# radiusxyz/delay-encryption-in-halo2

Measured on AMD Instinct MI355X. Metric: pallas_msm_mpoints_per_s_at_2^20, higher is better.
Workload: dtype u256; 1 GPU; 1 x MSM(2^20, pallas) + 1 x NTT(2^20, pasta_fp) per step per GPU, uniform scalars, SRS tables resident; configs_index=1, steps_in_flight=4, parallelism=single GPU, attempts=1

## Files before the change

### bindings/rust/dehalo-sys/src/lib.rs

```rust
#![allow(non_camel_case_types, non_upper_case_globals, clippy::too_many_arguments)]
#![no_std]

pub use core::ffi::{c_char, c_int, c_void};

pub type dehalo_status = c_int;
pub const DEHALO_OK: dehalo_status = 0;
pub const DEHALO_ERR_INVALID: dehalo_status = -1;
pub const DEHALO_ERR_NO_DEVICE: dehalo_status = -2;
pub const DEHALO_ERR_OOM: dehalo_status = -3;
pub const DEHALO_ERR_HIP: dehalo_status = -4;
pub const DEHALO_ERR_UNSUPPORTED: dehalo_status = -5;
pub const DEHALO_ERR_NOT_IN_TABLE: dehalo_status = -6;
pub const DEHALO_ERR_SHUFFLE: dehalo_status = -7;

pub type dehalo_curve = c_int;
pub const DEHALO_CURVE_BN254_G1: dehalo_curve = 0;
pub const DEHALO_CURVE_PALLAS: dehalo_curve = 1;
pub const DEHALO_CURVE_VESTA: dehalo_curve = 2;

pub type dehalo_field = c_int;
pub const DEHALO_FIELD_BN254_FR: dehalo_field = 0;
pub const DEHALO_FIELD_BN254_FQ: dehalo_field = 1;
pub const DEHALO_FIELD_PASTA_FP: dehalo_field = 2;
pub const DEHALO_FIELD_PASTA_FQ: dehalo_field = 3;
// ... 376 lines not shown
    pub fn dehalo_eval_polynomial_device(ctx: *mut dehalo_ctx, field: c_int, d_coeffs: *const u64, len: usize, stride_elems: usize, batch: usize, point: *const u64, d_out: *mut u64, stream: *mut c_void) -> c_int;
    pub fn dehalo_eval_polynomial_multi_device(ctx: *mut dehalo_ctx, field: c_int, d_polys: *const *const u64, count: usize, len: usize, points: *const u64, num_points: u32, d_out: *mut u64, stream: *mut c_void) -> c_int;
    pub fn dehalo_eval_polynomial_multi_masked_device(ctx: *mut dehalo_ctx, field: c_int, d_polys: *const *const u64, count: usize, len: usize, points: *const u64, num_points: u32, wanted: *const u8, d_out: *mut u64, stream: *mut c_void) -> c_int;
    pub fn dehalo_eval_polynomial_points_device(ctx: *mut dehalo_ctx, field: c_int, d_polys: *const *const u64, count: usize, len: usize, points: *const u64, num_points: u32, wanted: *const u32, d_out: *mut u64, stream: *mut c_void) -> c_int;
    pub fn dehalo_batch_invert(ctx: *mut dehalo_ctx, field: c_int, values: *mut u64, len: usize) -> c_int;
    pub fn dehalo_batch_invert_device(ctx: *mut dehalo_ctx, field: c_int, d_values: *mut u64, len: usize, stream: *mut c_void) -> c_int;
    pub fn dehalo_prefix_product_device(ctx: *mut dehalo_ctx, field: c_int, d_in: *const u64, len: usize, d_out: *mut u64, stream: *mut c_void) -> c_int;
    pub fn dehalo_grand_product(ctx: *mut dehalo_ctx, field: c_int, num: *const u64, den: *const u64, len: usize, z: *mut u64) -> c_int;
    pub fn dehalo_grand_product_device(ctx: *mut dehalo_ctx, field: c_int, d_num: *const u64, d_den: *const u64, len: usize, d_z: *mut u64, stream: *mut c_void) -> c_int;
    pub fn dehalo_grand_product_batch_device(ctx: *mut dehalo_ctx, field: c_int, d_num: *const u64, d_den: *const u64, len: usize, batch: usize, stride_elems: usize, d_z: *mut u64, stream: *mut c_void) -> c_int;
    pub fn dehalo_lincomb_device(ctx: *mut dehalo_ctx, field: c_int, d_cols: *const *const u64, coefs: *const u64, count: usize, len: usize, d_out: *mut u64, sub_const: *const u64, stream: *mut c_void) -> c_int;
    pub fn dehalo_scale_device(ctx: *mut dehalo_ctx, field: c_int, d_a: *mut u64, len: usize, pattern: *const u64, period: u32, d_factor: *const u64, stream: *mut c_void) -> c_int;
    pub fn dehalo_kate_division(ctx: *mut dehalo_ctx, field: c_int, a: *const u64, len: usize, point: *const u64, q: *mut u64) -> c_int;
    pub fn dehalo_kate_division_device(ctx: *mut dehalo_ctx, field: c_int, d_a: *const u64, len: usize, point: *const u64, d_q: *mut u64, stream: *mut c_void) -> c_int;
    pub fn dehalo_kate_division_batch_device(ctx: *mut dehalo_ctx, field: c_int, d_a: *const *const u64, len: usize, points: *const u64, d_q: *const *mut u64, count: usize, stream: *mut c_void) -> c_int;
    pub fn dehalo_vanishing_quotient_batch_device(ctx: *mut dehalo_ctx, field: c_int, d_a: *const *const u64, len: usize, points: *const *const u64, num_points: *const u32, d_q: *const *mut u64, count: usize, stream: *mut c_void) -> c_int;
    pub fn dehalo_convert_form_device(ctx: *mut dehalo_ctx, field: c_int, d_in: *const u64, d_out: *mut u64, n: usize, to_internal: c_int, stream: *mut c_void) -> c_int;
    pub fn dehalo_coset_ntt_form_device(ctx: *mut dehalo_ctx, field: c_int, d_coeffs: *const u64, log_n: u32, d_ext_out: *mut u64, log_ext: u32, omega_ext: *const u64, zeta: *const u64, batch: usize, form_flags: u32, stream: *mut c_void) -> c_int;
    pub fn dehalo_coset_intt_form_device(ctx: *mut dehalo_ctx, field: c_int, d_a: *mut u64, log_ext: u32, omega_ext_inv: *const u64, ext_n_inv: *const u64, zeta: *const u64, batch: usize, form_flags: u32, stream: *mut c_void) -> c_int;
    pub fn dehalo_graph_create(ctx: *mut dehalo_ctx, field: c_int, constants: *const u64, num_constants: u32, rotations: *const i32, num_rotations: u32, calcs: *const dehalo_calculation, num_calcs: u32, horner_parts: *const dehalo_source, num_horner_parts: u32, num_intermediates: u32, out: *mut *mut dehalo_graph) -> c_int;
    pub fn dehalo_graph_release(ctx: *mut dehalo_ctx, graph: *mut dehalo_graph) -> c_int;
    pub fn dehalo_graph_evaluate_device(ctx: *mut dehalo_ctx, graph: *const dehalo_graph, input: *const dehalo_eval_inputs, log_rows: u32, rot_scale: u32, d_previous: *const u64, d_out: *mut u64, stream: *mut c_void) -> c_int;
    pub fn dehalo_graph_evaluate_batch_device(ctx: *mut dehalo_ctx, graphs: *const *const dehalo_graph, count: u32, input: *const dehalo_eval_inputs, log_rows: u32, rot_scale: u32, d_outs: *const *mut u64, stream: *mut c_void) -> c_int;
    pub fn dehalo_permutation_h_device(ctx: *mut dehalo_ctx, field: c_int, input: *const dehalo_perm_inputs, log_rows: u32, rot_scale: u32, d_values: *mut u64, stream: *mut c_void) -> c_int;
    pub fn dehalo_lookup_h_device(ctx: *mut dehalo_ctx, field: c_int, input: *const dehalo_lookup_inputs, log_rows: u32, rot_scale: u32, d_values: *mut u64, stream: *mut c_void) -> c_int;
    pub fn dehalo_lookup_h_batch_device(ctx: *mut dehalo_ctx, field: c_int, input: *const dehalo_lookup_inputs, count: u32, log_rows: u32, rot_scale: u32, d_values: *mut u64, stream: *mut c_void) -> c_int;
    pub fn dehalo_shuffle_h_batch_device(ctx: *mut dehalo_ctx, field: c_int, input: *const dehalo_shuffle_inputs, count: u32, log_rows: u32, rot_scale: u32, d_values: *mut u64, stream: *mut c_void) -> c_int;
    pub fn dehalo_params_create(ctx: *mut dehalo_ctx, curve: c_int, k: u32, g: *const u64, g_lagrange: *const u64, g2: *const u8, s_g2: *const u8, out: *mut *mut dehalo_params) -> c_int;
    pub fn dehalo_params_setup(ctx: *mut dehalo_ctx, curve: c_int, k: u32, s: *const u64, out: *mut *mut dehalo_params) -> c_int;
    pub fn dehalo_params_ipa_create(ctx: *mut dehalo_ctx, curve: c_int, k: u32, g: *const u64, g_lagrange: *const u64, w: *const u64, u: *const u64, out: *mut *mut dehalo_params) -> c_int;
    pub fn dehalo_params_ipa_from_g(ctx: *mut dehalo_ctx, curve: c_int, k: u32, g: *const u64, w: *const u64, u: *const u64, out: *mut *mut dehalo_params) -> c_int;
    pub fn dehalo_params_ipa_size(params: *const dehalo_params) -> usize;
    pub fn dehalo_params_ipa_write(params: *const dehalo_params, out: *mut u8, cap: usize) -> c_int;
    pub fn dehalo_params_ipa_read(ctx: *mut dehalo_ctx, curve: c_int, bytes: *const u8, len: usize, out: *mut *mut dehalo_params) -> c_int;
    pub fn dehalo_params_scheme(params: *const dehalo_params) -> c_int;
    pub fn dehalo_params_fixed_base(params: *const dehalo_params) -> *const dehalo_fixed_base;
    pub fn dehalo_params_read(ctx: *mut dehalo_ctx, curve: c_int, bytes: *const u8, len: usize, out: *mut *mut dehalo_params) -> c_int;
    pub fn dehalo_params_size(params: *const dehalo_params) -> usize;
    pub fn dehalo_params_write(params: *const dehalo_params, out: *mut u8, cap: usize) -> c_int;
    pub fn dehalo_params_release(ctx: *mut dehalo_ctx, params: *mut dehalo_params) -> c_int;
    pub fn dehalo_params_commit_device(ctx: *mut dehalo_ctx, params: *const dehalo_params, d_polys: *const u64, batch: usize, lagrange: c_int, d_out_affine: *mut u64, stream: *mut c_void) -> c_int;
    pub fn dehalo_keygen(ctx: *mut dehalo_ctx, params: *const dehalo_params, cs: *const dehalo_constraint_system, fixed: *const u64, permutation_mapping: *const u64, selectors: *const *const u8, num_selectors: u32, flags: u32, out: *mut *mut dehalo_pk) -> c_int;
    pub fn dehalo_pk_read(ctx: *mut dehalo_ctx, curve: c_int, cs: *const dehalo_constraint_system, bytes: *const u8, len: usize, num_selectors: u32, out: *mut *mut dehalo_pk) -> c_int;
    pub fn dehalo_pk_size(pk: *const dehalo_pk) -> usize;
    pub fn dehalo_pk_write(ctx: *mut dehalo_ctx, pk: *const dehalo_pk, out: *mut u8, cap: usize) -> c_int;
    pub fn dehalo_vk_size(pk: *const dehalo_pk) -> usize;
    pub fn dehalo_vk_write(pk: *const dehalo_pk, out: *mut u8, cap: usize) -> c_int;
    pub fn dehalo_pk_set_transcript_repr(pk: *mut dehalo_pk, repr: *const u64) -> c_int;
    pub fn dehalo_pk_get_transcript_repr(pk: *const dehalo_pk, repr: *mut u64) -> c_int;
    pub fn dehalo_pk_info(pk: *const dehalo_pk, out: *mut u32) -> c_int;
    pub fn dehalo_pk_phases(pk: *const dehalo_pk, out: *mut u32) -> c_int;
    pub fn dehalo_pk_release(ctx: *mut dehalo_ctx, pk: *mut dehalo_pk) -> c_int;
    pub fn dehalo_rng_scalars(rng: *mut dehalo_rng, field: c_int, skip: u64, out: *mut u64, count: usize) -> c_int;
    pub fn dehalo_transcript_create(curve: c_int, out: *mut *mut dehalo_transcript) -> c_int;
    pub fn dehalo_transcript_common_scalar(t: *mut dehalo_transcript, scalar: *const u64) -> c_int;
    pub fn dehalo_transcript_write_scalar(t: *mut dehalo_transcript, scalar: *const u64) -> c_int;
    pub fn dehalo_transcript_write_point(t: *mut dehalo_transcript, affine_xy: *const u64) -> c_int;
    pub fn dehalo_transcript_squeeze_challenge(t: *mut dehalo_transcript, out: *mut u64) -> c_int;
    pub fn dehalo_transcript_len(t: *const dehalo_transcript) -> usize;
    pub fn dehalo_transcript_finalize(t: *const dehalo_transcript, out: *mut u8, cap: usize) -> c_int;
    pub fn dehalo_transcript_release(t: *mut dehalo_transcript);
    pub fn dehalo_ipa_open(ctx: *mut dehalo_ctx, params: *const dehalo_params, d_poly: *const u64, blind: *const u64, x3: *const u64, rng: *mut dehalo_rng, transcript: *mut dehalo_transcript) -> c_int;
    pub fn dehalo_prover_create(ctx: *mut dehalo_ctx, side_ctx: *mut dehalo_ctx, params: *const dehalo_params, pk: *const dehalo_pk, out: *mut *mut dehalo_prover) -> c_int;
    pub fn dehalo_prover_create_multi(ctx: *mut dehalo_ctx, side_ctx: *mut dehalo_ctx, params: *const dehalo_params, pk: *const dehalo_pk, num_circuits: u32, out: *mut *mut dehalo_prover) -> c_int;
    pub fn dehalo_prover_release(prover: *mut dehalo_prover) -> c_int;
    pub fn dehalo_prover_set_multiopen(prover: *mut dehalo_prover, multiopen: c_int) -> c_int;
    pub fn dehalo_prover_proof_size(prover: *const dehalo_prover) -> usize;
    pub fn dehalo_create_proof(prover: *mut dehalo_prover, advice: *const u64, instances: *const *const u64, instance_lens: *const usize, num_instance_columns: u32, rng: *mut dehalo_rng, transcript: *mut dehalo_transcript, flags: u32) -> c_int;
    pub fn dehalo_create_proof_multi(prover: *mut dehalo_prover, advice: *const *const u64, instances: *const *const u64, instance_lens: *const usize, num_instance_columns: u32, num_circuits: u32, rng: *mut dehalo_rng, transcript: *mut dehalo_transcript, flags: u32) -> c_int;
    pub fn dehalo_create_proof_phased(prover: *mut dehalo_prover, func: dehalo_advice_fn, user: *mut c_void, instances: *const *const u64, instance_lens: *const usize, num_instance_columns: u32, rng: *mut dehalo_rng, transcript: *mut dehalo_transcript, flags: u32) -> c_int;
    pub fn dehalo_check_witness(ctx: *mut dehalo_ctx, pk: *const dehalo_pk, advice: *const u64, instances: *const *const u64, instance_lens: *const usize, num_instance_columns: u32, permutation_mapping: *const u64, flags: u32, failures: *mut dehalo_check_failure, cap: usize, report: *mut dehalo_check_report) -> c_int;
    pub fn dehalo_check_witness_challenges(ctx: *mut dehalo_ctx, pk: *const dehalo_pk, advice: *const u64, instances: *const *const u64, instance_lens: *const usize, num_instance_columns: u32, permutation_mapping: *const u64, flags: u32, challenges: *const u64, num_challenges: u32, failures: *mut dehalo_check_failure, cap: usize, report: *mut dehalo_check_report) -> c_int;
    pub fn dehalo_prover_set_shard(prover: *mut dehalo_prover, rank: u32, world: u32, gather: dehalo_gather_fn, user: *mut c_void) -> c_int;
    pub fn dehalo_prover_last_timings(prover: *const dehalo_prover, out: *mut f64) -> c_int;
    pub fn dehalo_create_proofs(provers: *const *mut dehalo_prover, num_provers: u32, advice: *const *const u64, count: u32, rngs: *mut dehalo_rng, flags: u32, proofs_out: *const *mut u8, proof_cap: usize, proof_lens: *mut usize) -> c_int;
    pub fn dehalo_synthesize(input: *const dehalo_circuit_inputs, advice: *mut u64, fixed: *mut u64, mapping: *mut u64, selectors: *const *mut u8, info: *mut dehalo_synthesis_info) -> c_int;
    pub fn dehalo_create_proof_circuit(prover: *mut dehalo_prover, input: *const dehalo_circuit_inputs, info: *mut dehalo_synthesis_info, instances: *const *const u64, instance_lens: *const usize, num_instance_columns: u32, rng: *mut dehalo_rng, transcript: *mut dehalo_transcript) -> c_int;
    pub fn dehalo_create_proofs_circuit(provers: *const *mut dehalo_prover, num_provers: u32, inputs: *const dehalo_circuit_inputs, count: u32, rngs: *mut dehalo_rng, proofs_out: *const *mut u8, proof_cap: usize, proof_lens: *mut usize) -> c_int;
    pub fn dehalo_product_terms_device(ctx: *mut dehalo_ctx, field: c_int, input: *const dehalo_product_inputs, n: usize, d_num: *mut u64, d_den: *mut u64, stride_elems: usize, stream: *mut c_void) -> c_int;
    pub fn dehalo_timing_enable(ctx: *mut dehalo_ctx, on: c_int) -> c_int;
    pub fn dehalo_timing_reset(ctx: *mut dehalo_ctx) -> c_int;
    pub fn dehalo_timing_get(ctx: *mut dehalo_ctx, kernel_id: c_int, total_ms: *mut f64, count: *mut u64) -> c_int;
    pub fn dehalo_msm_last_shape(ctx: *mut dehalo_ctx, out: *mut u32) -> c_int;
    pub fn dehalo_field_info(field: c_int, out: *mut u64) -> c_int;
    pub fn dehalo_version() -> *const c_char;
}

pub const DEHALO_SYS_FUNCTIONS: usize = 132;
```

### delay-encryption-in-halo2_amd/_lib.py

```python
from __future__ import annotations

import ctypes as C
import os
import threading
from typing import Tuple, Optional, Sequence

import numpy as np

_HERE = os.path.dirname(os.path.abspath(__file__))
_LIB = None

SYMBOLS = [
    "dehalo_version", "dehalo_ctx_create", "dehalo_ctx_create_with_priority", "dehalo_ctx_destroy", "dehalo_last_error", "dehalo_ctx_synchronize", "dehalo_download", "dehalo_upload", "dehalo_ctx_stream", "dehalo_ctx_set_tuning",
    "dehalo_bases_register", "dehalo_bases_release", "dehalo_bases_len", "dehalo_bases_info",
    "dehalo_msm", "dehalo_msm_batch", "dehalo_msm_device", "dehalo_msm_device_affine", "dehalo_msm_last_shape", "dehalo_lookup_h_batch_device", "dehalo_product_terms_device", "dehalo_best_multiexp", "dehalo_to_affine", "dehalo_to_affine_device", "dehalo_point_sum_device",
    "dehalo_ntt", "dehalo_ntt_device", "dehalo_intt_scaled", "dehalo_coset_ntt", "dehalo_coset_intt",
    "dehalo_intt_scaled_device", "dehalo_lagrange_to_coeff_device", "dehalo_coset_ntt_device", "dehalo_coset_intt_device",
    "dehalo_field_op", "dehalo_field_op_device", "dehalo_timing_enable", "dehalo_timing_reset", "dehalo_timing_get",
    "dehalo_eval_polynomial", "dehalo_eval_polynomial_device", "dehalo_eval_polynomial_multi_device", "dehalo_eval_polynomial_multi_masked_device", "dehalo_eval_polynomial_points_device", "dehalo_batch_invert", "dehalo_batch_invert_device",
    "dehalo_prefix_product_device", "dehalo_grand_product", "dehalo_grand_product_device", "dehalo_grand_product_batch_device",
    "dehalo_permute_expression_pair", "dehalo_permute_expression_pair_device", "dehalo_permute_expression_pair_batch_device", "dehalo_permute_expression_pair_ptrs_device", "dehalo_permute_expression_pair_distinct_device", "dehalo_permute_expression_pair_ptrs_deferred_device",
    "dehalo_convert_form_device", "dehalo_coset_ntt_form_device", "dehalo_coset_intt_form_device",
    "dehalo_lincomb_device", "dehalo_scale_device", "dehalo_kate_division", "dehalo_kate_division_device", "dehalo_kate_division_batch_device", "dehalo_vanishing_quotient_batch_device",
    "dehalo_params_create", "dehalo_params_setup", "dehalo_bases_register_device", "dehalo_params_read", "dehalo_params_size", "dehalo_params_write", "dehalo_params_release", "dehalo_params_commit_device",
    "dehalo_create_proof_circuit", "dehalo_create_proofs_circuit", "dehalo_keygen", "dehalo_pk_read", "dehalo_pk_size", "dehalo_pk_write", "dehalo_vk_size", "dehalo_vk_write", "dehalo_pk_set_transcript_repr",
    "dehalo_pk_get_transcript_repr", "dehalo_pk_info", "dehalo_pk_release", "dehalo_rng_scalars", "dehalo_field_info", "dehalo_synthesize",
    "dehalo_transcript_create", "dehalo_transcript_common_scalar", "dehalo_transcript_write_scalar", "dehalo_transcript_write_point",
    "dehalo_transcript_squeeze_challenge", "dehalo_transcript_len", "dehalo_transcript_finalize", "dehalo_transcript_release",
    "dehalo_prover_create", "dehalo_prover_release", "dehalo_create_proof", "dehalo_prover_set_shard", "dehalo_prover_last_timings", "dehalo_create_proofs", "dehalo_prover_set_multiopen",
    "dehalo_params_ipa_create", "dehalo_params_scheme", "dehalo_generator_collapse_device", "dehalo_ipa_open", "dehalo_blind_commitments_device", "dehalo_prover_proof_size",
    "dehalo_g_to_lagrange_device", "dehalo_params_ipa_from_g", "dehalo_params_ipa_size", "dehalo_params_ipa_write", "dehalo_params_ipa_read",
    "dehalo_fixed_base_create", "dehalo_fixed_base_release", "dehalo_fixed_base_mul_device", "dehalo_fixed_base_blind_device", "dehalo_params_fixed_base",
    "dehalo_graph_create", "dehalo_graph_release", "dehalo_graph_evaluate_device", "dehalo_graph_evaluate_batch_device", "dehalo_permutation_h_device", "dehalo_lookup_h_device",
    "dehalo_check_witness", "dehalo_check_witness_challenges", "dehalo_create_proof_phased", "dehalo_pk_phases",
    "dehalo_prover_create_multi", "dehalo_create_proof_multi", "dehalo_shuffle_h_batch_device",
]

K_MSM_ACCUMULATE, K_MSM_SORT, K_MSM_REDUCE, K_NTT_PASS, K_POLY, K_EVAL_H = 0, 1, 2, 3, 4, 5


class CSource(C.Structure):
    _fields_ = [("kind", C.c_uint32), ("index", C.c_uint32), ("rotation", C.c_uint32)]


class CCalculation(C.Structure):
    _fields_ = [("op", C.c_uint32), ("a", CSource), ("b", CSource), ("parts_begin", C.c_uint32), ("parts_len", C.c_uint32), ("target", C.c_uint32)]


class CEvalInputs(C.Structure):
    _fields_ = [("fixed", C.POINTER(C.c_void_p)), ("num_fixed", C.c_uint32), ("advice", C.POINTER(C.c_void_p)), ("num_advice", C.c_uint32),
                ("instance", C.POINTER(C.c_void_p)), ("num_instance", C.c_uint32), ("challenges", C.c_void_p), ("num_challenges", C.c_uint32),
                ("beta", C.c_void_p), ("gamma", C.c_void_p), ("theta", C.c_void_p), ("y", C.c_void_p), ("form_flags", C.c_uint32)]


class CPermInputs(C.Structure):
    _fields_ = [("z", C.POINTER(C.c_void_p)), ("num_sets", C.c_uint32), ("columns", C.POINTER(C.c_void_p)), ("sigma", C.POINTER(C.c_void_p)),
                ("num_columns", C.c_uint32), ("chunk_len", C.c_uint32), ("last_rotation", C.c_int32),
                ("l0", C.c_void_p), ("l_last", C.c_void_p), ("l_active_row", C.c_void_p),
                ("beta", C.c_void_p), ("gamma", C.c_void_p), ("y", C.c_void_p), ("delta", C.c_void_p), ("beta_zeta", C.c_void_p), ("extended_omega", C.c_void_p),
                ("form_flags", C.c_uint32)]


class CLookupInputs(C.Structure):
    _fields_ = [("product_coset", C.c_void_p), ("permuted_input_coset", C.c_void_p), ("permuted_table_coset", C.c_void_p), ("table_value", C.c_void_p),
                ("l0", C.c_void_p), ("l_last", C.c_void_p), ("l_active_row", C.c_void_p), ("beta", C.c_void_p), ("gamma", C.c_void_p), ("y", C.c_void_p),
                ("form_flags", C.c_uint32)]


class CShuffleInputs(C.Structure):
    _fields_ = [("product_coset", C.c_void_p), ("input_value", C.c_void_p), ("shuffle_value", C.c_void_p),
                ("l0", C.c_void_p), ("l_last", C.c_void_p), ("l_active_row", C.c_void_p), ("y", C.c_void_p), ("form_flags", C.c_uint32)]


class CExprNode(C.Structure):
    _fields_ = [("kind", C.c_uint32), ("a", C.c_uint32), ("b", C.c_uint32), ("rotation", C.c_int32)]


class CColumnQuery(C.Structure):
    _fields_ = [("kind", C.c_uint32), ("index", C.c_uint32), ("rotation", C.c_int32)]


class CConstraintSystem(C.Structure):
    _fields_ = [("num_advice", C.c_uint32), ("num_fixed", C.c_uint32), ("num_instance", C.c_uint32), ("minimum_degree", C.c_uint32),
                ("nodes", C.POINTER(CExprNode)), ("num_nodes", C.c_uint32), ("constants", C.c_void_p), ("num_constants", C.c_uint32),
                ("gates", C.POINTER(C.c_uint32)), ("num_gates", C.c_uint32), ("lookup_lens", C.POINTER(C.c_uint32)), ("num_lookups", C.c_uint32),
                ("lookup_inputs", C.POINTER(C.c_uint32)), ("lookup_tables", C.POINTER(C.c_uint32)),
                ("permutation_columns", C.POINTER(CColumnQuery)), ("num_permutation_columns", C.c_uint32),
                ("advice_queries", C.POINTER(CColumnQuery)), ("num_advice_queries", C.c_uint32),
                ("fixed_queries", C.POINTER(CColumnQuery)), ("num_fixed_queries", C.c_uint32),
                ("instance_queries", C.POINTER(CColumnQuery)), ("num_instance_queries", C.c_uint32),
                ("advice_phases", C.c_void_p), ("challenge_phases", C.c_void_p), ("num_challenges", C.c_uint32),
                ("shuffle_lens", C.POINTER(C.c_uint32)), ("shuffle_inputs", C.POINTER(C.c_uint32)), ("shuffle_tables", C.POINTER(C.c_uint32)), ("num_shuffles", C.c_uint32)]


class CCircuitInputs(C.Structure):
    _fields_ = [("circuit", C.c_uint32), ("k", C.c_uint32), ("bits_len", C.c_uint32), ("exp_bits", C.c_uint32), ("n", C.c_void_p), ("x", C.c_void_p), ("e", C.c_uint64),
                ("message", C.c_void_p), ("message_len", C.c_uint32), ("key", C.c_void_p), ("t", C.c_uint32), ("rate", C.c_uint32), ("r_f", C.c_uint32), ("r_p", C.c_uint32)]


class CSynthesisInfo(C.Structure):
    _fields_ = [("rsa_rows", C.c_uint64), ("total_rows", C.c_uint64), ("rsa_result", C.c_uint64 * 128), ("cipher", C.c_uint64 * 12), ("cipher_len", C.c_uint32)]


RNG_FILL_FN = C.CFUNCTYPE(C.c_int, C.c_void_p, C.POINTER(C.c_uint64), C.c_size_t, C.c_uint64)
GATHER_FN = C.CFUNCTYPE(C.c_int, C.c_void_p, C.POINTER(C.c_uint64), C.c_uint32, C.POINTER(C.c_uint32), C.POINTER(C.c_uint32), C.c_uint32)
ADVICE_FN = C.CFUNCTYPE(C.c_int, C.c_void_p, C.c_uint32, C.POINTER(C.c_uint64), C.c_uint32, C.POINTER(C.c_void_p))


class CRng(C.Structure):
    _fields_ = [("kind", C.c_int), ("pcg_state", C.c_uint64 * 2), ("pcg_inc", C.c_uint64 * 2), ("fill", RNG_FILL_FN), ("user", C.c_void_p)]


class CProductInputs(C.Structure):
    _fields_ = [("columns", C.POINTER(C.c_void_p)), ("sigma", C.POINTER(C.c_void_p)), ("num_columns", C.c_uint32), ("chunk_len", C.c_uint32), ("omega_powers", C.c_void_p),
                ("beta", C.c_void_p), ("gamma", C.c_void_p), ("delta", C.c_void_p), ("set_factors", C.c_void_p), ("compressed_input", C.POINTER(C.c_void_p)),
                ("compressed_table", C.POINTER(C.c_void_p)), ("permuted_input", C.POINTER(C.c_void_p)), ("permuted_table", C.POINTER(C.c_void_p)), ("num_lookups", C.c_uint32)]


class CCheckFailure(C.Structure):
    _fields_ = [("kind", C.c_uint32), ("index", C.c_uint32), ("row", C.c_uint32), ("reserved", C.c_uint32)]


class CCheckReport(C.Structure):
    _fields_ = [("gate_failures", C.c_uint64), ("lookup_failures", C.c_uint64), ("copy_failures", C.c_uint64), ("rows", C.c_uint64), ("lookup_inputs", C.c_uint64),
                ("cells_in_cycles", C.c_uint64), ("written", C.c_uint64), ("shuffle_failures", C.c_uint64), ("shuffle_inputs", C.c_uint64)]


class DehaloError(RuntimeError):
    def __init__(self, code: int, msg: str):
        super().__init__("dehalo error %d: %s" % (code, msg))
        self.code = code


def library_path() -> str:
    return os.environ.get("DEHALO_LIBRARY") or os.path.join(_HERE, "libdehalo.so")


def load_library():
    global _LIB
    if _LIB is not None:
        return _LIB
    path = library_path()
    if not os.path.exists(path):
        raise DehaloError(-2, "libdehalo.so is not built (run `make` or __graft_entry__.build()); there is no CPU fallback")
    try:
        import torch
    except Exception:
        pass
    lib = C.CDLL(path)
    P, sz, u32, u64p = C.c_void_p, C.c_size_t, C.c_uint32, C.c_void_p
    lib.dehalo_version.restype = C.c_char_p
    lib.dehalo_last_error.restype = C.c_char_p
    lib.dehalo_last_error.argtypes = [P]
    lib.dehalo_ctx_create.argtypes = [C.c_int, C.POINTER(P)]
    lib.dehalo_ctx_create_with_priority.argtypes = [C.c_int, C.c_int, C.POINTER(P)]
    lib.dehalo_ctx_destroy.argtypes = [P]
    lib.dehalo_ctx_destroy.restype = None
    lib.dehalo_ctx_synchronize.argtypes = [P]
    lib.dehalo_download.argtypes = [P, P, C.c_size_t, P]
    lib.dehalo_upload.argtypes = [P, P, C.c_size_t, P]
    lib.dehalo_ctx_set_tuning.argtypes = [P, C.c_char_p, C.c_int]
    lib.dehalo_ctx_stream.argtypes = [P]
    lib.dehalo_ctx_stream.restype = C.c_void_p
    lib.dehalo_bases_register.argtypes = [P, C.c_int, u64p, sz, sz, C.c_int, C.c_int, C.POINTER(P)]
    lib.dehalo_bases_release.argtypes = [P, P]
    lib.dehalo_bases_len.argtypes = [P]
    lib.dehalo_bases_len.restype = sz
    lib.dehalo_bases_info.argtypes = [P, C.POINTER(C.c_uint32), C.POINTER(C.c_uint32), C.POINTER(C.c_int)]
    lib.dehalo_msm.argtypes = [P, P, u64p, sz, u64p]
    lib.dehalo_msm_batch.argtypes = [P, P, C.POINTER(C.c_void_p), sz, sz, u64p]
    lib.dehalo_msm_device.argtypes = [P, P, u64p, sz, sz, u64p, P]
    lib.dehalo_msm_device_affine.argtypes = [P, P, u64p, sz, sz, u64p, u64p, P]
    lib.dehalo_msm_last_shape.argtypes = [P, C.POINTER(C.c_uint32)]
    lib.dehalo_best_multiexp.argtypes = [P, C.c_int, u64p, u64p, sz, u64p]
    lib.dehalo_to_affine.argtypes = [P, C.c_int, u64p, sz, u64p]
    lib.dehalo_to_affine_device.argtypes = [P, C.c_int, u64p, sz, u64p, P]
    lib.dehalo_generator_collapse_device.argtypes = [P, C.c_int, u64p, sz, u64p, u64p, P]
    lib.dehalo_blind_commitments_device.argtypes = [P, C.c_int, u64p, u64p, sz, u64p, P]
    lib.dehalo_point_sum_device.argtypes = [P, C.c_int, u64p, sz, u64p, P]
    lib.dehalo_fixed_base_create.argtypes = [P, C.c_int, u64p, C.POINTER(P)]
    lib.dehalo_fixed_base_release.argtypes = [P, P]
    lib.dehalo_fixed_base_mul_device.argtypes = [P, P, u64p, sz, u64p, P]
    lib.dehalo_fixed_base_blind_device.argtypes = [P, P, u64p, u64p, sz, P]
    lib.dehalo_params_fixed_base.argtypes = [P]
    lib.dehalo_params_fixed_base.restype = C.c_void_p
    lib.dehalo_ntt.argtypes = [P, C.c_int, u64p, u32, u64p]
    lib.dehalo_ntt_device.argtypes = [P, C.c_int, u64p, u32, u64p, sz, P]
    lib.dehalo_intt_scaled.argtypes = [P, C.c_int, u64p, u32, u64p, u64p]
    lib.dehalo_coset_ntt.argtypes = [P, C.c_int, u64p, u32, u64p, u32, u64p, u64p]
    lib.dehalo_coset_intt.argtypes = [P, C.c_int, u64p, u32, u64p, u64p, u64p]
    lib.dehalo_intt_scaled_device.argtypes = [P, C.c_int, u64p, u32, u64p, u64p, sz, P]
    if hasattr(lib, "dehalo_lagrange_to_coeff_device"):
        lib.dehalo_lagrange_to_coeff_device.argtypes = [P, C.c_int, u64p, u64p, u32, u64p, u64p, sz, P]
    lib.dehalo_coset_ntt_device.argtypes = [P, C.c_int, u64p, u32, u64p, u32, u64p, u64p, sz, P]
    lib.dehalo_coset_intt_device.argtypes = [P, C.c_int, u64p, u32, u64p, u64p, u64p, sz, P]
    lib.dehalo_field_op.argtypes = [P, C.c_int, C.c_int, u64p, u64p, u64p, sz]
    lib.dehalo_field_op_device.argtypes = [P, C.c_int, C.c_int, u64p, u64p, u64p, sz, P]
    lib.dehalo_eval_polynomial.argtypes = [P, C.c_int, u64p, sz, u64p, u64p]
    lib.dehalo_eval_polynomial_device.argtypes = [P, C.c_int, u64p, sz, sz, sz, u64p, u64p, P]
    lib.dehalo_eval_polynomial_multi_device.argtypes = [P, C.c_int, C.POINTER(C.c_void_p), sz, sz, u64p, u32, u64p, P]
    lib.dehalo_eval_polynomial_points_device.argtypes = [P, C.c_int, C.POINTER(C.c_void_p), sz, sz, u64p, u32, C.POINTER(C.c_uint32), u64p, P]
    if hasattr(lib, "dehalo_eval_polynomial_multi_masked_device"):
        lib.dehalo_eval_polynomial_multi_masked_device.argtypes = [P, C.c_int, C.POINTER(C.c_void_p), sz, sz, u64p, u32, C.c_char_p, u64p, P]
    lib.dehalo_batch_invert.argtypes = [P, C.c_int, u64p, sz]
    lib.dehalo_batch_invert_device.argtypes = [P, C.c_int, u64p, sz, P]
    lib.dehalo_prefix_product_device.argtypes = [P, C.c_int, u64p, sz, u64p, P]
    lib.dehalo_grand_product.argtypes = [P, C.c_int, u64p, u64p, sz, u64p]
    lib.dehalo_grand_product_device.argtypes = [P, C.c_int, u64p, u64p, sz, u64p, P]
    lib.dehalo_grand_product_batch_device.argtypes = [P, C.c_int, u64p, u64p, sz, sz, sz, u64p, P]
    lib.dehalo_permute_expression_pair.argtypes = [P, C.c_int, u64p, u64p, sz, u64p, u64p]
    lib.dehalo_permute_expression_pair_device.argtypes = [P, C.c_int, u64p, u64p, sz, u64p, u64p, P]
    lib.dehalo_permute_expression_pair_batch_device.argtypes = [P, C.c_int, u64p, u64p, sz, sz, sz, u64p, u64p, P]
    if hasattr(lib, "dehalo_permute_expression_pair_ptrs_deferred_device"):
        lib.dehalo_permute_expression_pair_ptrs_deferred_device.argtypes = [P, C.c_int, C.POINTER(C.c_void_p), C.POINTER(C.c_void_p), sz, sz, C.POINTER(C.c_void_p), C.POINTER(C.c_void_p), P, P]
    if hasattr(lib, "dehalo_permute_expression_pair_distinct_device"):
        lib.dehalo_permute_expression_pair_distinct_device.argtypes = [P, C.c_int, C.POINTER(C.c_void_p), C.POINTER(C.c_void_p), sz, sz, C.POINTER(C.c_void_p), C.POINTER(C.c_void_p),
                                                                       C.POINTER(C.c_void_p), C.POINTER(C.c_void_p), C.POINTER(C.c_uint32), P, P]
    if hasattr(lib, "dehalo_permute_expression_pair_ptrs_device"):
        lib.dehalo_permute_expression_pair_ptrs_device.argtypes = [P, C.c_int, C.POINTER(C.c_void_p), C.POINTER(C.c_void_p), sz, sz, C.POINTER(C.c_void_p), C.POINTER(C.c_void_p), P]
    lib.dehalo_lincomb_device.argtypes = [P, C.c_int, C.POINTER(C.c_void_p), u64p, sz, sz, u64p, u64p, P]
    lib.dehalo_scale_device.argtypes = [P, C.c_int, u64p, sz, u64p, u32, u64p, P]
    lib.dehalo_kate_division.argtypes = [P, C.c_int, u64p, sz, u64p, u64p]
    lib.dehalo_kate_division_device.argtypes = [P, C.c_int, u64p, sz, u64p, u64p, P]
    lib.dehalo_kate_division_batch_device.argtypes = [P, C.c_int, C.POINTER(C.c_void_p), sz, u64p, C.POINTER(C.c_void_p), sz, P]
    lib.dehalo_vanishing_quotient_batch_device.argtypes = [P, C.c_int, C.POINTER(C.c_void_p), sz, C.POINTER(C.c_void_p), C.POINTER(C.c_uint32), C.POINTER(C.c_void_p), sz, P]
    lib.dehalo_convert_form_device.argtypes = [P, C.c_int, u64p, u64p, sz, C.c_int, P]
    lib.dehalo_coset_ntt_form_device.argtypes = [P, C.c_int, u64p, u32, u64p, u32, u64p, u64p, sz, u32, P]
    lib.dehalo_coset_intt_form_device.argtypes = [P, C.c_int, u64p, u32, u64p, u64p, u64p, sz, u32, P]
    lib.dehalo_graph_create.argtypes = [P, C.c_int, u64p, u32, C.POINTER(C.c_int32), u32, C.POINTER(CCalculation), u32, C.POINTER(CSource), u32, u32, C.POINTER(P)]
    lib.dehalo_graph_release.argtypes = [P, P]
    lib.dehalo_graph_evaluate_device.argtypes = [P, P, C.POINTER(CEvalInputs), u32, u32, u64p, u64p, P]
    lib.dehalo_graph_evaluate_batch_device.argtypes = [P, C.POINTER(C.c_void_p), u32, C.POINTER(CEvalInputs), u32, u32, C.POINTER(C.c_void_p), P]
    lib.dehalo_permutation_h_device.argtypes = [P, C.c_int, C.POINTER(CPermInputs), u32, u32, u64p, P]
    lib.dehalo_lookup_h_device.argtypes = [P, C.c_int, C.POINTER(CLookupInputs), u32, u32, u64p, P]
    if hasattr(lib, "dehalo_product_terms_device"):
        lib.dehalo_product_terms_device.argtypes = [P, C.c_int, C.POINTER(CProductInputs), sz, u64p, u64p, sz, P]
    lib.dehalo_lookup_h_batch_device.argtypes = [P, C.c_int, C.POINTER(CLookupInputs), u32, u32, u32, u64p, P]
    lib.dehalo_shuffle_h_batch_device.argtypes = [P, C.c_int, C.POINTER(CShuffleInputs), u32, u32, u32, u64p, P]
    PP = C.POINTER(P)
    lib.dehalo_params_create.argtypes = [P, C.c_int, u32, u64p, u64p, P, P, PP]
    lib.dehalo_params_setup.argtypes = [P, C.c_int, u32, u64p, PP]
    lib.dehalo_bases_register_device.argtypes = [P, C.c_int, u64p, C.c_size_t, C.c_int, C.c_int, PP]
    lib.dehalo_params_read.argtypes = [P, C.c_int, P, sz, PP]
    lib.dehalo_params_size.argtypes = [P]
    lib.dehalo_params_size.restype = sz
    lib.dehalo_params_write.argtypes = [P, P, sz]
    lib.dehalo_params_release.argtypes = [P, P]
    lib.dehalo_params_commit_device.argtypes = [P, P, u64p, sz, C.c_int, u64p, P]
    lib.dehalo_params_ipa_create.argtypes = [P, C.c_int, u32, u64p, u64p, u64p, u64p, PP]
    lib.dehalo_params_scheme.argtypes = [P]
    lib.dehalo_g_to_lagrange_device.argtypes = [P, C.c_int, u64p, u32, u64p, P]
    lib.dehalo_params_ipa_from_g.argtypes = [P, C.c_int, u32, u64p, u64p, u64p, PP]
    lib.dehalo_params_ipa_size.argtypes = [P]
    lib.dehalo_params_ipa_size.restype = sz
    lib.dehalo_params_ipa_write.argtypes = [P, P, sz]
    lib.dehalo_params_ipa_read.argtypes = [P, C.c_int, P, sz, PP]
# ... 112 lines not shown
            self.handle = None

    def __enter__(self):
        return self

    def __exit__(self, *exc):
        self.close()

    def _check(self, rc: int):
        if rc != 0:
            raise DehaloError(rc, self.lib.dehalo_last_error(self.handle).decode())

    def synchronize(self):
        self._check(self.lib.dehalo_ctx_synchronize(self.handle))

    def download(self, d_src: int, count: int, width: int = 4) -> np.ndarray:
        out = np.empty((count, width), dtype=np.uint64)
        self._check(self.lib.dehalo_download(self.handle, d_src, out.nbytes, out.ctypes.data))
        return out

    def upload(self, host, dtype=None):
        import torch

        a = np.ascontiguousarray(host)
        assert a.dtype.itemsize in (8, 4, 1), "upload: 64-bit words (field elements, indices), 32-bit words or bytes"
        if dtype is None:
            dtype = {8: torch.int64, 4: torch.int32, 1: torch.uint8}[a.dtype.itemsize]
        out = torch.empty(a.shape, dtype=dtype, device=torch.device("cuda", self.device))
        self._check(self.lib.dehalo_upload(self.handle, a.ctypes.data, a.nbytes, out.data_ptr()))
        return out

    def download_tensor(self, t) -> np.ndarray:
        assert t.is_contiguous() and t.element_size() == 8
        out = np.empty(tuple(t.shape), dtype=np.uint64)
        self._check(self.lib.dehalo_download(self.handle, t.data_ptr(), out.nbytes, out.ctypes.data))
        return out

    def set_tuning(self, key: str, value: int):
        self._check(self.lib.dehalo_ctx_set_tuning(self.handle, key.encode(), value))

    def torch_stream_obj(self):
        self.torch_stream()
        return self._tstream

    def torch_stream(self):
        import torch

        if getattr(self, "_tstream", None) is None:
            self._tstream = torch.cuda.ExternalStream(self.lib.dehalo_ctx_stream(self.handle))
        return torch.cuda.stream(self._tstream)

    def register_bases(self, curve: int, affine_xy, window_bits: int = 0, precompute: bool = True) -> Bases:
        a = _u64(affine_xy, 8)
        h = C.c_void_p()
        self._check(self.lib.dehalo_bases_register(self.handle, curve, _ptr(a), a.shape[0], 64, window_bits, int(precompute), C.byref(h)))
        return Bases(self, h, curve, a.shape[0])

    def msm(self, bases: Bases, scalars) -> np.ndarray:
        s = _u64(scalars, 4)
        out = np.zeros(12, dtype=np.uint64)
        self._check(self.lib.dehalo_msm(self.handle, bases.handle, _ptr(s), s.shape[0], _ptr(out)))
        return out

    def msm_batch(self, bases: Bases, columns: Sequence) -> np.ndarray:
        cols = [_u64(c, 4) for c in columns]
        n = cols[0].shape[0] if cols else 0
        assert all(c.shape[0] == n for c in cols)
        ptrs = (C.c_void_p * len(cols))(*[c.ctypes.data for c in cols])
        out = np.zeros((len(cols), 12), dtype=np.uint64)
        self._check(self.lib.dehalo_msm_batch(self.handle, bases.handle, ptrs, n, len(cols), _ptr(out)))
        return out

    def msm_device(self, bases: Bases, d_scalars: int, length: int, batch: int, d_out: int, stream: int = 0):
        self._check(self.lib.dehalo_msm_device(self.handle, bases.handle, d_scalars, length, batch, d_out, stream or None))

    def msm_device_affine(self, bases: Bases, d_scalars: int, length: int, batch: int, d_out_jacobian: int, d_out_affine: int, stream: int = 0):
        self._check(self.lib.dehalo_msm_device_affine(self.handle, bases.handle, d_scalars, length, batch, d_out_jacobian or None, d_out_affine, stream or None))

    def msm_last_shape(self) -> dict:
        out = (C.c_uint32 * 6)()
        self._check(self.lib.dehalo_msm_last_shape(self.handle, out))
        return {"merge_light": out[0], "merge_32": out[1], "merge_wave": out[2], "merge_block": out[3], "points_per_lane": out[4], "pairs": out[5]}

    def best_multiexp(self, curve: int, scalars, affine_xy) -> np.ndarray:
        s, a = _u64(scalars, 4), _u64(affine_xy, 8)
        if s.shape[0] != a.shape[0]:
            raise ValueError("best_multiexp: coeffs.len() != bases.len()")
        out = np.zeros(12, dtype=np.uint64)
        self._check(self.lib.dehalo_best_multiexp(self.handle, curve, _ptr(s), _ptr(a), s.shape[0], _ptr(out)))
        return out

    def to_affine(self, curve: int, jacobian) -> np.ndarray:
        j = _u64(jacobian, 12)
        out = np.zeros((j.shape[0], 8), dtype=np.uint64)
        self._check(self.lib.dehalo_to_affine(self.handle, curve, _ptr(j), j.shape[0], _ptr(out)))
        return out

    def point_sum_device(self, curve: int, d_jacobian: int, count: int, d_out: int, stream: int = 0):
        self._check(self.lib.dehalo_point_sum_device(self.handle, curve, d_jacobian, count, d_out, stream or None))

    def generator_collapse_device(self, curve: int, d_affine: int, length: int, challenge, d_out: int, stream: int = 0):
        ch = np.ascontiguousarray(challenge, dtype=np.uint64).reshape(4)
        self._check(self.lib.dehalo_generator_collapse_device(self.handle, curve, d_affine, length, ch.ctypes.data, d_out, stream or None))

    def g_to_lagrange(self, curve: int, d_g: int, k: int, d_out: Optional[int] = None, stream: int = 0):
        self._check(self.lib.dehalo_g_to_lagrange_device(self.handle, curve, d_g, k, d_g if d_out is None else d_out, stream or None))

    def blind_commitments_device(self, curve: int, d_jacobian: int, d_blinds: int, count: int, d_w_affine: int, stream: int = 0):
        self._check(self.lib.dehalo_blind_commitments_device(self.handle, curve, d_jacobian or None, d_blinds or None, count, d_w_affine or None, stream or None))

    def fixed_base(self, curve: int, affine_xy) -> FixedBase:
        a = np.ascontiguousarray(affine_xy, dtype=np.uint64).reshape(8)
        h = C.c_void_p()
        self._check(self.lib.dehalo_fixed_base_create(self.handle, curve, _ptr(a), C.byref(h)))
        return FixedBase(self, h, curve)

    def to_affine_device(self, curve: int, d_jacobian: int, count: int, d_affine: int, stream: int = 0):
        self._check(self.lib.dehalo_to_affine_device(self.handle, curve, d_jacobian, count, d_affine, stream or None))

    def ntt(self, field: int, a, log_n: int, omega) -> np.ndarray:
        a = np.array(a, dtype=np.uint64).reshape(-1, 4)
        if a.shape[0] != 1 << log_n:
            raise ValueError("best_fft: a.len() != 1 << log_n")
        self._check(self.lib.dehalo_ntt(self.handle, field, _ptr(a), log_n, _ptr(_u64(omega, 4))))
        return a

    def intt_scaled(self, field: int, a, log_n: int, omega_inv, n_inv) -> np.ndarray:
        a = np.array(a, dtype=np.uint64).reshape(-1, 4)
        if a.shape[0] != 1 << log_n:
            raise ValueError("a.len() != 1 << log_n")
        self._check(self.lib.dehalo_intt_scaled(self.handle, field, _ptr(a), log_n, _ptr(_u64(omega_inv, 4)), _ptr(_u64(n_inv, 4))))
        return a

    def coset_ntt(self, field: int, coeffs, log_n: int, log_ext: int, omega_ext, zeta) -> np.ndarray:
        c = _u64(coeffs, 4)
        if c.shape[0] != 1 << log_n:
            raise ValueError("coeffs.len() != 1 << log_n")
        out = np.zeros((1 << log_ext, 4), dtype=np.uint64)
        self._check(self.lib.dehalo_coset_ntt(self.handle, field, _ptr(c), log_n, _ptr(out), log_ext, _ptr(_u64(omega_ext, 4)), _ptr(_u64(zeta, 4))))
        return out

    def coset_intt(self, field: int, a, log_ext: int, omega_ext_inv, ext_n_inv, zeta) -> np.ndarray:
        a = np.array(a, dtype=np.uint64).reshape(-1, 4)
        if a.shape[0] != 1 << log_ext:
            raise ValueError("a.len() != 1 << log_ext")
        self._check(self.lib.dehalo_coset_intt(self.handle, field, _ptr(a), log_ext, _ptr(_u64(omega_ext_inv, 4)), _ptr(_u64(ext_n_inv, 4)),
                                               _ptr(_u64(zeta, 4))))
        return a

    def ntt_device(self, field: int, d_a: int, log_n: int, omega, batch: int = 1, stream: int = 0):
        self._check(self.lib.dehalo_ntt_device(self.handle, field, d_a, log_n, _ptr(_u64(omega, 4)), batch, stream or None))

    def intt_scaled_device(self, field: int, d_a: int, log_n: int, omega_inv, n_inv, batch: int = 1, stream: int = 0):
        self._check(self.lib.dehalo_intt_scaled_device(self.handle, field, d_a, log_n, _ptr(_u64(omega_inv, 4)), _ptr(_u64(n_inv, 4)), batch, stream or None))

    def lagrange_to_coeff_device(self, field: int, d_values: int, d_coeffs: int, log_n: int, omega_inv, n_inv, batch: int = 1, stream: int = 0):
        self._check(self.lib.dehalo_lagrange_to_coeff_device(self.handle, field, d_values, d_coeffs, log_n, _ptr(_u64(omega_inv, 4)), _ptr(_u64(n_inv, 4)), batch, stream or None))

    def coset_ntt_device(self, field: int, d_coeffs: int, log_n: int, d_ext: int, log_ext: int, omega_ext, zeta, batch: int = 1, stream: int = 0):
        self._check(self.lib.dehalo_coset_ntt_device(self.handle, field, d_coeffs, log_n, d_ext, log_ext, _ptr(_u64(omega_ext, 4)), _ptr(_u64(zeta, 4)), batch,
                                                     stream or None))

    def convert_form_device(self, field: int, d_in: int, d_out: int, n: int, to_internal: bool, stream: int = 0):
        self._check(self.lib.dehalo_convert_form_device(self.handle, field, d_in, d_out, n, int(to_internal), stream or None))

    def coset_ntt_form_device(self, field: int, d_coeffs: int, log_n: int, d_ext: int, log_ext: int, omega_ext, zeta, batch: int, form_flags: int, stream: int = 0):
# ... 282 lines not shown
```

### delay-encryption-in-halo2_amd/csrc/capi.hip

```cpp
#include <algorithm>
#include <atomic>
#include <initializer_list>

#include <map>
#include <memory>

#include "evalh_types.hpp"
#include "hostfield.hpp"
#include "internal.hpp"
#include "msm_plan.hpp"

namespace {

const FieldOps* field_ops(int field) {
    static const FieldOps* const ops[] = {&bn254_fr_field_ops(), &bn254_fq_field_ops(), &pasta_fp_field_ops(), &pasta_fq_field_ops()};
    static_assert(DEHALO_FIELD_BN254_FR == 0 && DEHALO_FIELD_BN254_FQ == 1 && DEHALO_FIELD_PASTA_FP == 2 && DEHALO_FIELD_PASTA_FQ == 3, "field ids");
    return field >= 0 && field < 4 ? ops[field] : nullptr;
}
const CurveOps* curve_ops(int curve) {
    static const CurveOps* const ops[] = {&bn254_curve_ops(), &pallas_curve_ops(), &vesta_curve_ops()};
    static_assert(DEHALO_CURVE_BN254_G1 == 0 && DEHALO_CURVE_PALLAS == 1 && DEHALO_CURVE_VESTA == 2, "curve ids");
    return curve >= 0 && curve < 3 ? ops[curve] : nullptr;
}
int unknown_field(dehalo_ctx* ctx) { return dh_fail(ctx, DEHALO_ERR_INVALID, "unknown field id"); }
// ... 273 lines not shown
        hipDeviceProp_t prop;
        if (hipGetDeviceProperties(&prop, device) != hipSuccess) return DEHALO_ERR_NO_DEVICE;
        if (strncmp(prop.gcnArchName, "gfx950", 6) != 0) return DEHALO_ERR_NO_DEVICE;
        if (hipSetDevice(device) != hipSuccess) return DEHALO_ERR_NO_DEVICE;
        std::unique_ptr<dehalo_ctx> ctx(new dehalo_ctx());
        ctx->device = device;
        ctx->num_cus = prop.multiProcessorCount > 0 ? prop.multiProcessorCount : 256;
        {
            int least = 0, greatest = 0;
            (void)hipDeviceGetStreamPriorityRange(&least, &greatest);
            const int prio = priority > 0 ? greatest : (priority < 0 ? least : 0);
            static const int cu_parts = [] { const char* e = DH_EXPERIMENT_ENV("DEHALO_CU_PARTITION"); return e ? atoi(e) : 0; }();
            static std::atomic<int> cu_next{0};
            hipError_t e;
            hipStream_t st = nullptr;
            if (cu_parts > 1 && cu_parts <= 16) {
                const int part = cu_next.fetch_add(1) % cu_parts, ncu = ctx->num_cus, per = ncu / cu_parts;
                std::vector<uint32_t> mask((ncu + 31) / 32, 0u);
                static const bool interleave = DH_EXPERIMENT_ENV("DEHALO_CU_PARTITION_INTERLEAVE") != nullptr;
                for (int cu = 0; cu < ncu; cu++) {
                    const bool mine = interleave ? (cu % cu_parts) == part : (cu / per) == part;
                    if (mine) mask[cu / 32] |= 1u << (cu % 32);
                }
                e = hipExtStreamCreateWithCUMask(&st, (uint32_t)mask.size(), mask.data());
                if (e == hipSuccess) ctx->num_cus = per;
            } else
            e = priority == 0 ? hipStreamCreateWithFlags(&st, hipStreamNonBlocking)
                              : hipStreamCreateWithPriority(&st, hipStreamNonBlocking, prio);
            if (e != hipSuccess) return DEHALO_ERR_HIP;
            ctx->stream.reset(st);
        }
        if (const char* e = DH_EXPERIMENT_ENV("DEHALO_MSM_ACC_MIN_LAYERS")) ctx->msm_acc_min_layers = std::max(1, std::min(4, atoi(e)));
        if (const char* e = DH_EXPERIMENT_ENV("DEHALO_HOST_SPIN_US")) ctx->host_wait_spin_us = std::max(0, std::min(1000000, atoi(e)));
        if (const char* e = DH_EXPERIMENT_ENV("DEHALO_MSM_ACC_BLOCK")) ctx->msm_acc_block = atoi(e) == 768 ? 768 : 128;
        if (const char* e = DH_EXPERIMENT_ENV("DEHALO_MSM_ACC_POINTS")) ctx->msm_acc_points = std::max(0, std::min(4096, atoi(e)));
        *out = ctx.release();
        return 0;
    });
}

void dehalo_ctx_destroy(dehalo_ctx* ctx) {
    if (!ctx) return;
    (void)hipSetDevice(ctx->device);
    (void)hipDeviceSynchronize();
    delete ctx;
}

const char* dehalo_last_error(const dehalo_ctx* ctx) {
    if (!ctx) return "null context";
    static thread_local std::string copy;
    try {
        std::lock_guard<std::mutex> lk(const_cast<dehalo_ctx*>(ctx)->err_mu);
        copy = ctx->err;
    } catch (...) {
        return "out of host memory copying the last error";
    }
    return copy.c_str();
}

int dehalo_ctx_set_tuning(dehalo_ctx* ctx, const char* key, int value) {
    if (!ctx || !key) return DEHALO_ERR_INVALID;
    return dh_guard(ctx, [&]() -> int {
        std::lock_guard<std::recursive_mutex> lk(ctx->mu);
        if (!strcmp(key, "msm_acc_points")) {
            if (value < 0 || value > 4096) return dh_fail(ctx, DEHALO_ERR_INVALID, "msm_acc_points must be in [0, 4096]");
            ctx->msm_acc_points = value;
            return 0;
        }
        if (!strcmp(key, "msm_acc_waves")) {
            if (value < 1 || value > 4) return dh_fail(ctx, DEHALO_ERR_INVALID, "msm_acc_waves must be in [1, 4]");
            ctx->msm_acc_waves = value;
            return 0;
        }
        if (!strcmp(key, "host_wait_spin_us")) {
            if (value < 0 || value > 1000000) return dh_fail(ctx, DEHALO_ERR_INVALID, "host_wait_spin_us must be in [0, 1000000]");
            ctx->host_wait_spin_us = value;
            return 0;
        }
        if (!strcmp(key, "msm_sort_block")) {
            if (value != 512 && value != 1024) return dh_fail(ctx, DEHALO_ERR_INVALID, "msm_sort_block must be 512 or 1024");
            ctx->msm_sort_block = value;
            return 0;
        }
        if (!strcmp(key, "msm_acc_block")) {
            if (value != 128 && value != 768) return dh_fail(ctx, DEHALO_ERR_INVALID, "msm_acc_block must be 128 or 768");
            ctx->msm_acc_block = value;
            return 0;
        }
        if (!strcmp(key, "ntt_full_table_log")) {
            if (value < 0 || value > 30) return dh_fail(ctx, DEHALO_ERR_INVALID, "ntt_full_table_log must be in [0, 30]");
            ctx->ntt_full_table_log = value;
            return 0;
        }
        return dh_fail(ctx, DEHALO_ERR_INVALID, std::string("unknown tuning key: ") + key);
    });
}

void* dehalo_ctx_stream(dehalo_ctx* ctx) { return ctx ? (void*)ctx->stream.get() : nullptr; }

int dehalo_ctx_synchronize(dehalo_ctx* ctx) {
    if (!ctx) return DEHALO_ERR_INVALID;
    return dh_guard(ctx, [&]() -> int {
        HIP_TRY(ctx, hipStreamSynchronize(ctx->stream.get()));
        return 0;
    });
}

int dehalo_download(dehalo_ctx* ctx, const void* d_src, size_t bytes, void* host_dst) {
    if (!ctx) return DEHALO_ERR_INVALID;
    return dh_guard(ctx, [&]() -> int {
        if ((!d_src || !host_dst) && bytes) return dh_fail(ctx, DEHALO_ERR_INVALID, "download: null argument");
        (void)hipSetDevice(ctx->device);
        if (bytes) TRY(dh_d2h(ctx, host_dst, d_src, bytes, ctx->stream.get()));
        HIP_TRY(ctx, dh_stream_wait(ctx, ctx->stream.get()));
        return 0;
    });
}

int dehalo_upload(dehalo_ctx* ctx, const void* host_src, size_t bytes, void* d_dst) {
    if (!ctx) return DEHALO_ERR_INVALID;
    return dh_guard(ctx, [&]() -> int {
        if ((!host_src || !d_dst) && bytes) return dh_fail(ctx, DEHALO_ERR_INVALID, "upload: null argument");
        (void)hipSetDevice(ctx->device);
        {
            HostPin pin(host_src, bytes);
            TRY(dh_h2d(ctx, d_dst, host_src, bytes, ctx->stream.get()));
            HIP_TRY(ctx, hipStreamSynchronize(ctx->stream.get()));
        }
        return 0;
    });
}

int dehalo_bases_register(dehalo_ctx* ctx, int curve, const uint64_t* affine_xy, size_t n, size_t stride_bytes, int window_bits, int precompute,
                          dehalo_bases** out) {
    return register_entry(ctx, curve, affine_xy, n, stride_bytes, window_bits, precompute, out, false);
}

int dehalo_bases_register_device(dehalo_ctx* ctx, int curve, const uint64_t* d_affine_xy, size_t n, int window_bits, int precompute, dehalo_bases** out) {
    return register_entry(ctx, curve, d_affine_xy, n, 64, window_bits, precompute, out, true);
}

int dehalo_bases_release(dehalo_ctx* ctx, dehalo_bases* bases) {
    if (!ctx || !bases) return DEHALO_ERR_INVALID;
    return dh_guard(ctx, [&] {
        std::lock_guard<std::recursive_mutex> lk(ctx->mu);
        (void)hipSetDevice(ctx->device);
        (void)hipDeviceSynchronize();
        delete bases;
        return 0;
    });
}

size_t dehalo_bases_len(const dehalo_bases* bases) { return bases ? bases->n : 0; }

int dehalo_bases_info(const dehalo_bases* bases, uint32_t* window_bits, uint32_t* windows, int* precomputed) {
    if (!bases) return DEHALO_ERR_INVALID;
    if (window_bits) *window_bits = bases->c;
    if (windows) *windows = bases->W;
    if (precomputed) *precomputed = bases->precomp;
    return 0;
}

int dehalo_msm_device(dehalo_ctx* ctx, const dehalo_bases* bases, const uint64_t* d_scalars, size_t len, size_t batch, uint64_t* d_out_jacobian,
                      void* stream) {
    if (!bases || (!d_scalars && len) || !d_out_jacobian) return dh_fail(ctx, DEHALO_ERR_INVALID, "msm: null argument");
    if (len > bases->n) return dh_fail(ctx, DEHALO_ERR_INVALID, "msm: more scalars than registered bases");
// ... 724 lines not shown
        return dh_fail(ctx, DEHALO_ERR_INVALID, "product_terms: incomplete permutation inputs");
    if (in->num_lookups && (!in->compressed_input || !in->compressed_table || !in->permuted_input || !in->permuted_table))
        return dh_fail(ctx, DEHALO_ERR_INVALID, "product_terms: incomplete lookup inputs");
    if (in->num_columns > 256 || in->num_lookups > 256) return dh_fail(ctx, DEHALO_ERR_INVALID, "product_terms: too many columns");
    if (stride_elems < n) return dh_fail(ctx, DEHALO_ERR_INVALID, "product_terms: stride shorter than the columns");
    return field_device(ctx, field, stream, [&](const FieldOps& f, hipStream_t s) { return f.product_terms(ctx, in, n, (fe*)d_num, (fe*)d_den, stride_elems, s); });
}

int dehalo_lookup_h_batch_device(dehalo_ctx* ctx, int field, const dehalo_lookup_inputs* in, uint32_t count, uint32_t log_rows, uint32_t rot_scale,
                                 uint64_t* d_values, void* stream) {
    if (!in || !d_values || count == 0) return dh_fail(ctx, DEHALO_ERR_INVALID, "lookup_h_batch: null argument");
    if (count > 8) return dh_fail(ctx, DEHALO_ERR_INVALID, "lookup_h_batch: more than 8 lookups in one call");
    for (uint32_t l = 0; l < count; l++) {
        const dehalo_lookup_inputs& q = in[l];
        if (!q.product_coset || !q.permuted_input_coset || !q.permuted_table_coset || !q.table_value || !q.l0 || !q.l_last || !q.l_active_row || !q.beta ||
            !q.gamma || !q.y)
            return dh_fail(ctx, DEHALO_ERR_INVALID, "lookup_h_batch: null argument");
        if (q.l0 != in[0].l0 || q.l_last != in[0].l_last || q.l_active_row != in[0].l_active_row || q.form_flags != in[0].form_flags ||
            memcmp(q.beta, in[0].beta, 32) || memcmp(q.gamma, in[0].gamma, 32) || memcmp(q.y, in[0].y, 32))
            return dh_fail(ctx, DEHALO_ERR_INVALID, "lookup_h_batch: the lookups of one call share l0 / l_last / l_active_row, the challenges and the form flags");
    }
    if (log_rows > 30) return dh_fail(ctx, DEHALO_ERR_INVALID, "lookup_h: log_rows > 30");
    return field_device(ctx, field, stream, [&](const FieldOps& f, hipStream_t s) { return f.lookup_h_batch(ctx, in, count, log_rows, rot_scale, (fe*)d_values, s); });
}

int dehalo_shuffle_h_batch_device(dehalo_ctx* ctx, int field, const dehalo_shuffle_inputs* in, uint32_t count, uint32_t log_rows, uint32_t rot_scale,
                                  uint64_t* d_values, void* stream) {
    if (!in || !d_values || count == 0) return dh_fail(ctx, DEHALO_ERR_INVALID, "shuffle_h_batch: null argument");
    if (count > 8) return dh_fail(ctx, DEHALO_ERR_INVALID, "shuffle_h_batch: more than 8 shuffles in one call");
    for (uint32_t j = 0; j < count; j++) {
        const dehalo_shuffle_inputs& q = in[j];
        if (!q.product_coset || !q.input_value || !q.shuffle_value || !q.l0 || !q.l_last || !q.l_active_row || !q.y)
            return dh_fail(ctx, DEHALO_ERR_INVALID, "shuffle_h_batch: null argument");
        if (q.l0 != in[0].l0 || q.l_last != in[0].l_last || q.l_active_row != in[0].l_active_row || q.form_flags != in[0].form_flags || memcmp(q.y, in[0].y, 32))
            return dh_fail(ctx, DEHALO_ERR_INVALID, "shuffle_h_batch: the shuffles of one call share l0 / l_last / l_active_row, y and the form flags");
    }
    if (log_rows > 30) return dh_fail(ctx, DEHALO_ERR_INVALID, "shuffle_h_batch: log_rows > 30");
    return field_device(ctx, field, stream, [&](const FieldOps& f, hipStream_t s) { return f.shuffle_h_batch(ctx, in, count, log_rows, rot_scale, (fe*)d_values, s); });
}

int dehalo_timing_enable(dehalo_ctx* ctx, int on) {
    if (!ctx) return DEHALO_ERR_INVALID;
    return dh_guard(ctx, [&]() -> int {
        std::lock_guard<std::recursive_mutex> lk(ctx->mu);
        ctx->timing = on != 0;
        return 0;
    });
}

static int timing_collect(dehalo_ctx* ctx) {
    (void)hipSetDevice(ctx->device);
    for (auto& r : ctx->regions) {
        HIP_TRY(ctx, hipEventSynchronize(r.b.get()));
        float ms = 0;
        HIP_TRY(ctx, hipEventElapsedTime(&ms, r.a.get(), r.b.get()));
        ctx->timing_ms[r.kernel_id] += ms;
        ctx->timing_cnt[r.kernel_id] += 1;
    }
    ctx->regions.clear();
    return 0;
}

int dehalo_timing_reset(dehalo_ctx* ctx) {
    if (!ctx) return DEHALO_ERR_INVALID;
    return dh_guard(ctx, [&]() -> int {
        std::lock_guard<std::recursive_mutex> lk(ctx->mu);
        TRY(timing_collect(ctx));
        for (int i = 0; i < DEHALO_K_COUNT; i++) { ctx->timing_ms[i] = 0; ctx->timing_cnt[i] = 0; }
        return 0;
    });
}

int dehalo_timing_get(dehalo_ctx* ctx, int kernel_id, double* total_ms, uint64_t* count) {
    if (!ctx || kernel_id < 0 || kernel_id >= DEHALO_K_COUNT || !total_ms || !count) return DEHALO_ERR_INVALID;
    return dh_guard(ctx, [&]() -> int {
        std::lock_guard<std::recursive_mutex> lk(ctx->mu);
        TRY(timing_collect(ctx));
        *total_ms = ctx->timing_ms[kernel_id];
        *count = ctx->timing_cnt[kernel_id];
        return 0;
    });
}

int dehalo_msm_last_shape(dehalo_ctx* ctx, uint32_t out[6]) {
    if (!ctx || !out) return DEHALO_ERR_INVALID;
    return dh_guard(ctx, [&]() -> int {
        std::lock_guard<std::recursive_mutex> lk(ctx->mu);
        (void)hipSetDevice(ctx->device);
        memset(out, 0, 6 * sizeof(uint32_t));
        if (!ctx->ws_counters.p) return 0;
        HIP_TRY(ctx, hipStreamSynchronize(ctx->stream.get()));
        uint32_t raw[10];
        HIP_TRY(ctx, hipMemcpy(raw, ctx->ws_counters.p, sizeof(raw), hipMemcpyDeviceToHost));
        out[0] = raw[0] + raw[1] + raw[2]; out[1] = raw[3]; out[2] = raw[4]; out[3] = raw[6]; out[4] = raw[8]; out[5] = raw[9];
        return 0;
    });
}

}

int dh_graph_create_roots(dehalo_ctx* ctx, int field, const uint64_t* constants, uint32_t num_constants, const int32_t* rotations, uint32_t num_rotations,
                          const dehalo_calculation* calcs, uint32_t num_calcs, const dehalo_source* horner_parts, uint32_t num_horner_parts, uint32_t num_intermediates,
                          const uint32_t* root_of, uint32_t num_roots, dehalo_graph** out) {
    if (ctx && num_calcs && !root_of) return dh_fail(ctx, DEHALO_ERR_INVALID, "graph_create: null root table");
    return graph_create_impl(ctx, field, constants, num_constants, rotations, num_rotations, calcs, num_calcs, horner_parts, num_horner_parts, num_intermediates, root_of,
                             num_roots, out);
}
```

### delay-encryption-in-halo2_amd/csrc/internal.hpp

```cpp
#pragma once
#include <hip/hip_runtime.h>

#include <algorithm>
#include <cstdint>
#include <cstdlib>
#include <cstring>
#include <map>
#include <chrono>
#include <mutex>
#include <string>
#include <thread>
#include <vector>

#include "../../include/dehalo.h"
#include "ec.cuh"
#include "experiment_env.hpp"
#include "guard.hpp"
#include "owners.hpp"

using DevMem = DevArray<fe>;

struct HostStage {
    static constexpr size_t CHUNK = 4u << 20;
    static constexpr size_t DIRECT_MAX = 64u << 10;
    std::mutex mu;
    Pinned<void> buf[2];
    Event ev[2];
    bool busy[2] = {false, false};
};

struct TwiddleEntry {
    int field;
    uint32_t log_n;
    int form;
    uint64_t omega[4];
    uint64_t len;
    DevMem tw;
};

struct TimedRegion {
    int kernel_id;
    Event a, b;
};

struct dehalo_ctx {
    int device = 0;
    int num_cus = 256;
    Stream stream;
    std::string err;
    std::mutex err_mu;
    std::recursive_mutex mu;
    DevBuf ws_scalars, ws_out, ws_count, ws_counters, ws_off, ws_records, ws_merge_lists, ws_merge_parts, ws_bhist, ws_pcount, ws_pairs, ws_bsum, ws_idx, ws_partial0, ws_buckets,
        ws_contrib, ws_tree, ws_bred_cnt, ws_gsums, ws_ntt_scratch, ws_ntt_io, ws_ntt_io2, ws_fop[3], ws_tmp_bases, ws_poly[5], ws_poly_io[3], ws_evh[4], ws_lookup, ws_gfft, ws_check[3];
    std::vector<TwiddleEntry> twiddles;
    affine_t* msm_affine_out = nullptr;
    int msm_acc_points = 48;
    int msm_acc_waves = 3;
    int host_wait_spin_us = 400;
    int msm_acc_min_layers = 4;
    int msm_sort_block = 1024;
    int msm_acc_block = 128;
    int ntt_full_table_log = 0;
    HostStage stage;
    bool timing = false;
    std::vector<TimedRegion> regions;
    double timing_ms[DEHALO_K_COUNT] = {};
    uint64_t timing_cnt[DEHALO_K_COUNT] = {};
};

struct dehalo_bases {
    int curve;
    size_t n;
    uint32_t c, W;
    int precomp;
    DevArray<affine_t> table;
};

struct dehalo_fixed_base {
    int curve;
    DevArray<affine_t> table;
};

inline int dh_fail(dehalo_ctx* ctx, int code, const char* msg) noexcept {
    if (ctx) try {
        std::lock_guard<std::mutex> lk(ctx->err_mu);
        ctx->err = msg;
    } catch (...) {}
    return code;
}
inline int dh_fail(dehalo_ctx* ctx, int code, const std::string& msg) noexcept { return dh_fail(ctx, code, msg.c_str()); }

template <class Body>
int dh_guard(dehalo_ctx* ctx, Body&& body) noexcept {
    return dh_guard_noting([ctx](const char* msg) { dh_fail(ctx, DEHALO_ERR_INVALID, msg); }, body);
}

inline hipStream_t pick_stream(dehalo_ctx* ctx, void* stream) { return stream ? (hipStream_t)stream : ctx->stream.get(); }
inline hipStream_t dh_ctx_stream(dehalo_ctx* ctx) { return ctx->stream.get(); }

template <class Body>
int dh_device(dehalo_ctx* ctx, void* stream, Body&& body) noexcept {
    if (!ctx) return DEHALO_ERR_INVALID;
    return dh_guard(ctx, [&]() -> int {
        std::lock_guard<std::recursive_mutex> lk(ctx->mu);
        (void)hipSetDevice(ctx->device);
        return body(pick_stream(ctx, stream));
    });
}

inline hipError_t dh_func_lds(dehalo_ctx* ctx, const void* fn, int bytes) {
    static std::mutex mu;
    static std::map<std::pair<int, const void*>, int> have;
    std::lock_guard<std::mutex> lk(mu);
    int& cur = have[std::make_pair(ctx->device, fn)];
    if (cur >= bytes) return hipSuccess;
    const hipError_t e = hipFuncSetAttribute(fn, hipFuncAttributeMaxDynamicSharedMemorySize, bytes);
    if (e == hipSuccess) cur = bytes;
    return e;
}

inline int dh_ensure(dehalo_ctx* ctx, DevBuf& b, size_t bytes) { return b.ensure(ctx, bytes); }

inline bool dh_host_locked(const void* ptr, size_t bytes) {
    {
        HostPinRegistry& reg = host_pin_registry();
        std::lock_guard<std::mutex> lk(reg.mu);
        const uintptr_t a = (uintptr_t)ptr, b = a + bytes;
        for (auto& e : reg.entries)
            if (e.a <= a && b <= e.b) return true;
    }
    hipPointerAttribute_t at;
    if (hipPointerGetAttributes(&at, ptr) == hipSuccess) return at.type == hipMemoryTypeHost;
    (void)hipGetLastError();
    return false;
}

inline int dh_stage_init(dehalo_ctx* ctx) {
    HostStage& st = ctx->stage;
    for (int i = 0; i < 2; i++) {
        if (!st.buf[i]) HIP_TRY(ctx, make_pinned(st.buf[i], HostStage::CHUNK));
        if (!st.ev[i]) HIP_TRY(ctx, make_event(st.ev[i], hipEventDisableTiming));
    }
// ... 203 lines not shown
```

### delay-encryption-in-halo2_amd/csrc/msm.cuh

```cuda
#pragma once
#include <algorithm>
#include <cstdlib>
#include <cstdio>
#include <vector>

#include "ec29.cuh"
#include "internal.hpp"
#include "msm_plan.hpp"

#ifndef MSM_ACC_WAVES_ATTR
#ifdef MSM_ACC_CAP
#define MSM_ACC_WAVES_ATTR __attribute__((amdgpu_waves_per_eu(MSM_ACC_CAP, MSM_ACC_CAP)))
#else
#define MSM_ACC_WAVES_ATTR __attribute__((amdgpu_waves_per_eu(4, 4)))
#endif
#endif
#ifdef MSM_HIST_VGPR64
#define MSM_HIST_ATTR __attribute__((amdgpu_num_vgpr(64)))
#else
#define MSM_HIST_ATTR
#endif

#ifndef MSM_TAIL_PRIO
#define MSM_TAIL_PRIO 0
#endif
FP_DEV void msm_tail_prio() {
#if MSM_TAIL_PRIO > 0
    __builtin_amdgcn_s_setprio(MSM_TAIL_PRIO);
#endif
}

FP_DEV u32 merge2_class(u32 S) { return S <= 2 ? 0u : S <= 4 ? 1u : S <= 8 ? 2u : S <= 64 ? 3u : S <= MERGE2_CHUNK ? 4u : 5u; }

FP_DEV bool fe_is_zero_words(const fe& a) { return (a.v[0] | a.v[1] | a.v[2] | a.v[3] | a.v[4] | a.v[5] | a.v[6] | a.v[7]) == 0; }

template <class FS, class Fn>
FP_DEV void for_each_digit(const fe& mont_scalar, u32 c, u32 w_lo, u32 w_hi, Fn f) {
    if (fe_is_zero_words(mont_scalar)) return;
    fe s = f_from_mont<FS>(mont_scalar);
    u32 bits = 0;
#pragma unroll
    for (int i = 0; i < 8; i++) if (s.v[i]) bits = 32u * i + (32u - (u32)__clz((int)s.v[i]));
    const u32 w_end = min(w_hi, (bits + c - 1) / c + 1);
    const u32 mask = (1u << c) - 1, halfv = 1u << (c - 1);
    u32 carry = 0;
    for (u32 w = 0; w < w_end; w++) {
        u32 raw = (s.v[0] & mask) + carry;
#pragma unroll
        for (int i = 0; i < 7; i++) s.v[i] = (s.v[i] >> c) | (s.v[i + 1] << (32 - c));
        s.v[7] >>= c;
        bool neg = raw > halfv;
        carry = neg ? 1u : 0u;
        u32 mag = neg ? (1u << c) - raw : raw;
        if (mag != 0 && w >= w_lo) f(w, mag - 1, neg);
    }
}

struct DigitStream {
    fe s;
    u32 carry, c, mask, halfv;
    template <class FS>
    FP_DEV void init(const fe& mont_scalar, u32 c_) {
        s = f_from_mont<FS>(mont_scalar);
        c = c_; mask = (1u << c) - 1; halfv = 1u << (c - 1); carry = 0;
    }
    FP_DEV bool exhausted() const { return carry == 0 && fe_is_zero_words(s); }
    FP_DEV void next(u32& bucket, bool& neg) {
        u32 raw = (s.v[0] & mask) + carry;
#pragma unroll
        for (int i = 0; i < 7; i++) s.v[i] = (s.v[i] >> c) | (s.v[i + 1] << (32 - c));
        s.v[7] >>= c;
        neg = raw > halfv;
        carry = neg ? 1u : 0u;
        u32 mag = neg ? (1u << c) - raw : raw;
        bucket = mag - 1;
    }
};

FP_DEV bool wave_value_groups(const fe& s, bool active, u32 lane, u32 max_groups, u32& leader, u32& cnt, u32& rank) {
    unsigned long long rem = __ballot(active);
    leader = lane; cnt = 1; rank = 0;
    for (u32 n = 0; rem; n++) {
        if (n == max_groups) return false;
        const int ld = __ffsll((long long)rem) - 1;
        bool eq = active;
#pragma unroll
        for (int w = 0; w < 8; w++) eq &= s.v[w] == (u32)__shfl((int)s.v[w], ld);
        const unsigned long long m = __ballot(eq);
        if (eq) { leader = (u32)ld; cnt = (u32)__popcll(m); rank = (u32)__popcll(m & ((1ull << lane) - 1)); }
        rem &= ~m;
    }
    return true;
}

template <class FS, bool PACK16>
__global__ __launch_bounds__(MSM_SORT_THREADS) MSM_HIST_ATTR void k_msm_hist(MsmGeom g, const fe* scalars, u32* bh, u32* pc) {
    msm_tail_prio();
    extern __shared__ u32 lhist[];
    const u32 bat = blockIdx.z;
    const u32 w_lo = g.G == 1 ? 0 : blockIdx.y * g.wb, w_hi = g.G == 1 ? g.W : min(g.W, w_lo + g.wb);
    const u32 ng = g.G == 1 ? 1 : w_hi - w_lo, grp0 = g.G == 1 ? 0 : w_lo;
    for (u32 b = threadIdx.x; b < (PACK16 ? ng * g.nb / 2 : ng * g.nb); b += blockDim.x) lhist[b] = 0;
    __syncthreads();
    const fe* sc = scalars + (u64)bat * g.n;
    const u32 per = (g.n + g.slices - 1) / g.slices;
    const u32 beg = blockIdx.x * per, end = min(beg + per, g.n);
    const bool one = g.G == 1;
    for (u32 i0 = beg + threadIdx.x; i0 < end; i0 += 4 * blockDim.x) {
        fe s4[4];
#pragma unroll
        for (int j = 0; j < 4; j++)
            if (i0 + j * blockDim.x < end) s4[j] = f_load(&sc[i0 + j * blockDim.x]);
#pragma unroll
        for (int j = 0; j < 4; j++) {
            const bool valid = i0 + j * blockDim.x < end;
            u32 gl, weight, grank;
            const bool grouped = wave_value_groups(s4[j], valid, threadIdx.x & 63, 4, gl, weight, grank);
            if (!grouped) weight = 1;
            const bool counts = grouped ? valid && (threadIdx.x & 63) == gl : valid;
            if (counts)
                for_each_digit<FS>(s4[j], g.c, w_lo, w_hi, [&](u32 w, u32 bucket, bool) {
                    const u32 slot = (one ? 0u : (w - w_lo) * g.nb) + bucket;
                    if (PACK16) atomicAdd(&lhist[slot >> 1], weight << ((slot & 1u) << 4));
                    else atomicAdd(&lhist[slot], weight);
                });
        }
    }
    __syncthreads();
    const u32 sub = msm_sub_bits(g.c), P = g.nb >> sub;
    for (u32 gi = 0; gi < ng; gi++) {
        const u64 gidx = (u64)bat * g.G + grp0 + gi;
        const u32* lh = lhist + (PACK16 ? gi * g.nb / 2 : gi * g.nb);
        if (PACK16) {
            u32* out = bh + ((gidx * g.slices + blockIdx.x) * g.nb) / 2;
            for (u32 w = threadIdx.x; w < g.nb / 2; w += blockDim.x) out[w] = lh[w];
        } else {
            u32* out = bh + (gidx * g.slices + blockIdx.x) * g.nb;
            for (u32 b = threadIdx.x; b < g.nb; b += blockDim.x) out[b] = lh[b];
        }
        u32* pout = pc + (gidx * g.slices + blockIdx.x) * P;
        const u32 nsub = 1u << sub, lane = threadIdx.x & 63;
        for (u32 q = threadIdx.x >> 6; q < P; q += blockDim.x >> 6) {
            u32 sum = 0;
            if (PACK16) {
                for (u32 w = lane; w < nsub / 2; w += 64) { const u32 x = lh[(q << sub) / 2 + w]; sum += (x & 0xffffu) + (x >> 16); }
            } else {
                for (u32 b = lane; b < nsub; b += 64) sum += lh[(q << sub) + b];
            }
#pragma unroll
            for (int d = 32; d > 0; d >>= 1) sum += __shfl_down(sum, d);
            if (lane == 0) pout[q] = sum;
        }
    }
}

template <bool SRC16>
FP_DEV u32 colscan_one(u32 nb, u32 slices, u32 total_buckets, u32* bh, const unsigned short* src16, u32* count, u32 gb) {
    if (gb >= total_buckets) return 0;
    u32 grp = gb / nb, b = gb - grp * nb;
    u32* col = bh + (u64)grp * slices * nb + b;
    const unsigned short* col16 = SRC16 ? src16 + (u64)grp * slices * nb + b : nullptr;
    u32 run = 0;
    u32 k = 0;
    for (; k + 16 <= slices; k += 16) {
        u32 v[16];
#pragma unroll
        for (int j = 0; j < 16; j++) v[j] = SRC16 ? (u32)col16[(u64)(k + j) * nb] : col[(u64)(k + j) * nb];
#pragma unroll
        for (int j = 0; j < 16; j++) {
            col[(u64)(k + j) * nb] = run;
            run += v[j];
        }
    }
    for (; k < slices; k++) {
        u32 v = SRC16 ? (u32)col16[(u64)k * nb] : col[(u64)k * nb];
        col[(u64)k * nb] = run;
        run += v;
    }
    if (count) count[gb] = run;
    return run;
}
static __global__ __launch_bounds__(SCAN_THREADS) void k_msm_colscan(u32 nb, u32 slices, u32 total_buckets, u32* bh, const unsigned short* bh16, u32* count, u32 blocks_a, u32 P,
                                                                     u32 total_parts, u32* pc, u32* bsum_items, u32* bsum_tasks, u32* merge_counters) {
    msm_tail_prio();
    if (blockIdx.x == 0 && threadIdx.x < MSM_MERGE_COUNTERS) merge_counters[threadIdx.x] = 0;
    if (blockIdx.x >= blocks_a) {
        colscan_one<false>(P, slices, total_parts, pc, nullptr, nullptr, (blockIdx.x - blocks_a) * blockDim.x + threadIdx.x);
        return;
    }
    const u32 gb0 = blockIdx.x * blockDim.x + threadIdx.x;
    const u32 v = bh16 ? colscan_one<true>(nb, slices, total_buckets, bh, bh16, count, gb0) : colscan_one<false>(nb, slices, total_buckets, bh, nullptr, count, gb0);
    u32 si = v, st = v ? 1u : 0u;
#pragma unroll
    for (int d = 32; d > 0; d >>= 1) { si += __shfl_down(si, d); st += __shfl_down(st, d); }
    __shared__ u32 w_i[SCAN_THREADS / 64], w_t[SCAN_THREADS / 64];
    if ((threadIdx.x & 63) == 0) { w_i[threadIdx.x >> 6] = si; w_t[threadIdx.x >> 6] = st; }
    __syncthreads();
    if (threadIdx.x == 0) {
        u32 a = 0, b = 0;
        for (u32 w = 0; w < SCAN_THREADS / 64; w++) { a += w_i[w]; b += w_t[w]; }
        bsum_items[blockIdx.x] = a; bsum_tasks[blockIdx.x] = b;
    }
}

static __global__ __launch_bounds__(SCAN_THREADS) void k_scan_offsets(const u32* cnt, u32 total, const u32* bsum_items, const u32* bsum_tasks, u32 nblocks, u32* geo, u32 resident,
                                                                      u32 lmax, u32 lcap, u32 kmin, u32* off, u32* nrank, u32* rbeg, u32* rend, u32* lists, u32 cap) {
    msm_tail_prio();
    __shared__ u32 s_i[SCAN_THREADS], s_t[SCAN_THREADS];
    __shared__ u32 w4[4][SCAN_THREADS / 64];
    const u32 tid = threadIdx.x, lane = tid & 63, wave = tid >> 6;
    u32 bi = 0, bt = 0, ti = 0;
    for (u32 j = tid; j < nblocks; j += SCAN_THREADS) {
        const u32 a = bsum_items[j];
        ti += a;
        if (j < blockIdx.x) { bi += a; bt += bsum_tasks[j]; }
    }
#pragma unroll
    for (int d = 32; d > 0; d >>= 1) { bi += __shfl_down(bi, d); bt += __shfl_down(bt, d); ti += __shfl_down(ti, d); }
    if (lane == 0) { w4[0][wave] = bi; w4[1][wave] = bt; w4[2][wave] = ti; }
    const u32 idx = blockIdx.x * SCAN_THREADS + tid;
    const u32 vi = idx < total ? cnt[idx] : 0, vt = vi ? 1u : 0u;
    s_i[tid] = vi; s_t[tid] = vt;
    __syncthreads();
    bi = 0; bt = 0; ti = 0;
    for (u32 w = 0; w < SCAN_THREADS / 64; w++) { bi += w4[0][w]; bt += w4[1][w]; ti += w4[2][w]; }
    const u64 M = ti;
    u64 L;
    if (lcap) {
        u64 k = kmin;
        while (M > k * resident * lcap) k += k < 4 ? 1 : 2;
        L = max((u64)4, (M + k * resident - 1) / (k * resident));
    } else {
        const u64 rounds = max((u64)1, (M + (u64)resident * lmax - 1) / ((u64)resident * lmax));
        L = (M + rounds * resident - 1) / (rounds * resident);
        L = min((u64)lmax, max((u64)4, L));
    }
    if (blockIdx.x == 0 && tid == 0) { geo[0] = (u32)L; geo[1] = (u32)M; }
    for (u32 d = 1; d < SCAN_THREADS; d <<= 1) {
        const u32 ai = tid >= d ? s_i[tid - d] : 0, at = tid >= d ? s_t[tid - d] : 0;
        __syncthreads();
        s_i[tid] += ai; s_t[tid] += at;
        __syncthreads();
    }
    const u32 ri = bi + s_i[tid] - vi, rt = bt + s_t[tid] - vt;
    u32 S = 0;
    if (idx < total) {
        off[idx] = ri; nrank[idx] = rt;
        const u32 b0 = (u32)(ri / L) + rt;
        const u32 b1 = vi ? (u32)((ri + vi - 1) / L) + rt + 1 : b0;
        rbeg[idx] = b0;
        rend[idx] = b1;
        S = b1 - b0;
        if (idx + 1 == total) { off[total] = ri + vi; nrank[total] = rt + vt; }
    }
    if (!lists) return;
    u32* counters = geo - MSM_MERGE_COUNTERS;
    const u32 cls = S <= 1 ? 8u : merge2_class(S);
    __shared__ u32 wcnt[5][SCAN_THREADS / 64], cbase[5];
    unsigned long long mine = 0;
    for (u32 c = 0; c < 5; c++) {
        const unsigned long long mask = __ballot(cls == c);
        if (cls == c) mine = mask;
        if (lane == 0) wcnt[c][wave] = (u32)__popcll(mask);
    }
    __syncthreads();
    if (tid < 5) {
        u32 tot = 0;
        for (u32 w = 0; w < SCAN_THREADS / 64; w++) tot += wcnt[tid][w];
        cbase[tid] = tot ? atomicAdd(&counters[tid], tot) : 0u;
    }
    __syncthreads();
    if (cls < 5) {
        u32 pos = cbase[cls] + (u32)__popcll(mine & ((1ull << lane) - 1));
        for (u32 w = 0; w < wave; w++) pos += wcnt[cls][w];
        lists[(size_t)cls * cap + pos] = idx;
    }
    if (cls == 5u) {
        const u32 parts = (S + MERGE2_CHUNK - 1) / MERGE2_CHUNK;
        const u32 slot = atomicAdd(&counters[6], 1u), first = atomicAdd(&counters[5], parts);
        u32* hb = lists + (size_t)6 * cap + 4 * (size_t)slot;
        hb[0] = idx; hb[1] = first; hb[2] = parts; hb[3] = 0;
        for (u32 p = 0; p < parts; p++) {
            lists[(size_t)5 * cap + 2 * (size_t)(first + p)] = slot;
            lists[(size_t)5 * cap + 2 * (size_t)(first + p) + 1] = p;
        }
    }
}

template <class FS>
__global__ __launch_bounds__(MSM_SORT_THREADS) void k_msm_part(MsmGeom g, const fe* scalars, const u32* off, const u32* pc, unsigned long long* pairs, u32 lists) {
    msm_tail_prio();
    extern __shared__ __align__(8) unsigned char part_smem[];
    const u32 bat = blockIdx.z;
    const u32 sub = msm_sub_bits(g.c), P = g.nb >> sub, submask = (1u << sub) - 1;
    const u32 w_lo = g.G == 1 ? 0 : blockIdx.y * g.wb, w_hi = g.G == 1 ? g.W : min(g.W, w_lo + g.wb);
    const u32 ng = g.G == 1 ? 1 : w_hi - w_lo, grp0 = g.G == 1 ? 0 : w_lo;
    const u32 PT = ng * P;
    const bool one = g.G == 1;
    const u32 wave = threadIdx.x >> 6, lane = threadIdx.x & 63, nwaves = blockDim.x >> 6;
    u32* pcur = reinterpret_cast<u32*>(part_smem);
    unsigned char* wbase = part_smem + 4 * lists + (size_t)wave * MSM_PART_WAVE_LDS(lists);
    unsigned long long* stage = reinterpret_cast<unsigned long long*>(wbase);
    u32* lcnt = reinterpret_cast<u32*>(wbase + 512 * 8);
    u32* lbase = lcnt + lists;
    u32* lcur = lbase + lists;
    u32* gbase = lcur + lists;
    unsigned short* stageq = reinterpret_cast<unsigned short*>(gbase + lists);
    for (u32 qq = threadIdx.x; qq < PT; qq += blockDim.x) {
        const u32 gi = qq / P, q = qq - gi * P;
        const u64 gidx = (u64)bat * g.G + grp0 + gi;
        pcur[qq] = off[gidx * g.nb + (q << sub)] + pc[(gidx * g.slices + blockIdx.x) * P + q];
    }
    __syncthreads();
    const fe* sc = scalars + (u64)bat * g.n;
    const u32 per = (g.n + g.slices - 1) / g.slices;
    const u32 beg = blockIdx.x * per, end = min(beg + per, g.n);
    (void)nwaves;
    fe s_next;
    if (beg + wave * 64 + lane < end) s_next = f_load(&sc[beg + wave * 64 + lane]);
    for (u32 i0 = beg + wave * 64; i0 < end; i0 += blockDim.x) {
        const u32 i = i0 + lane;
        const bool have = i < end;
        const fe s_cur = s_next;
        if (i + blockDim.x < end) s_next = f_load(&sc[i + blockDim.x]);
        const bool nonzero = have && !fe_is_zero_words(s_cur);
        const unsigned long long actm = __ballot(nonzero);
        if (actm == 0) continue;
        DigitStream ds;
        if (nonzero) ds.template init<FS>(s_cur, g.c);
        {
            u32 gl, gcnt, grank;
            if (__popcll(actm) > 1 && wave_value_groups(s_cur, nonzero, lane, 4, gl, gcnt, grank)) {
                for (u32 w = 0; w < w_hi; w++) {
                    if (__ballot(nonzero && !ds.exhausted()) == 0) break;
                    u32 bk = 0xffffffffu; bool ng1 = false;
                    if (nonzero) ds.next(bk, ng1);
                    const bool put = nonzero && w >= w_lo && bk != 0xffffffffu;
                    const u32 q = put ? (one ? 0u : (w - w_lo) * P) + (bk >> sub) : 0u;
                    u32 g0 = 0;
                    if (put && lane == gl) g0 = atomicAdd(&pcur[q], gcnt);
                    g0 = (u32)__shfl((int)g0, (int)gl);
                    const u32 tidx = one ? w * g.table_n + i : i;
                    if (put) pairs[g0 + grank] = ((unsigned long long)(bk & submask) << 32) | (tidx | (ng1 ? 0x80000000u : 0u));
                }
                continue;
            }
        }
        for (u32 w0 = 0; w0 < w_hi; w0 += 8) {
            if (__ballot(nonzero && !ds.exhausted()) == 0) break;
            u32 bk[8];
            bool ng8[8];
#pragma unroll
            for (int j = 0; j < 8; j++) {
                bk[j] = 0xffffffffu; ng8[j] = false;
                if (nonzero && w0 + j < w_hi) {
                    ds.next(bk[j], ng8[j]);
                    if (w0 + j < w_lo) bk[j] = 0xffffffffu;
                }
            }
            if (w0 + 8 <= w_lo) continue;
            for (u32 q = lane; q < PT; q += 64) lcnt[q] = 0;
            __builtin_amdgcn_wave_barrier();
#pragma unroll
            for (int j = 0; j < 8; j++)
                if (bk[j] != 0xffffffffu) atomicAdd(&lcnt[(one ? 0u : (w0 + j - w_lo) * P) + (bk[j] >> sub)], 1u);
            __builtin_amdgcn_wave_barrier();
            u32 run = 0;
            for (u32 q0 = 0; q0 < PT; q0 += 64) {
                const u32 q = q0 + lane;
                const u32 v = q < PT ? lcnt[q] : 0;
                u32 x = v;
#pragma unroll
                for (int d = 1; d < 64; d <<= 1) { u32 y = __shfl_up(x, d); if ((int)lane >= d) x += y; }
                if (q < PT) {
                    lbase[q] = run + x - v; lcur[q] = run + x - v;
                    gbase[q] = v ? atomicAdd(&pcur[q], v) : 0u;
                }
                run += __shfl(x, 63);
            }
            __builtin_amdgcn_wave_barrier();
#pragma unroll
            for (int j = 0; j < 8; j++)
                if (bk[j] != 0xffffffffu) {
                    const u32 q = (one ? 0u : (w0 + j - w_lo) * P) + (bk[j] >> sub);
                    const u32 pos = atomicAdd(&lcur[q], 1u);
                    const u32 tidx = one ? (w0 + j) * g.table_n + i : i;
                    stage[pos] = ((unsigned long long)(bk[j] & submask) << 32) | (tidx | (ng8[j] ? 0x80000000u : 0u));
                    stageq[pos] = (unsigned short)q;
                }
            __builtin_amdgcn_wave_barrier();
            for (u32 e = lane; e < run; e += 64) {
                const u32 q = stageq[e];
                pairs[gbase[q] + (e - lbase[q])] = stage[e];
            }
            __builtin_amdgcn_wave_barrier();
        }
    }
}

static __global__ __launch_bounds__(256) void k_msm_bucket(u32 nb, u32 c, u32 slices, const u32* off, const u32* bh, const u32* pc,
                                                          const unsigned long long* pairs, u32* idx_out, u32 per_block) {
    msm_tail_prio();
    __shared__ u32 lcur[512], lfirst[512];
    const u32 sub = msm_sub_bits(c), P = nb >> sub, nsub = 1u << sub;
    const u32 chunks = (slices + per_block - 1) / per_block;
    const u64 gidx = blockIdx.y;
    u32 p, ch;
    if ((P & 7) == 0) {
        u32 xcd = blockIdx.x & 7, j = blockIdx.x >> 3;
        p = xcd + 8 * (j / chunks);
        ch = j % chunks;
    } else {
        p = blockIdx.x / chunks;
        ch = blockIdx.x % chunks;
    }
    const u32 k0 = ch * per_block, k1 = min(k0 + per_block, slices);
    const u32* goff = off + gidx * nb + ((u64)p << sub);
    const u32* rel = bh + (gidx * slices + k0) * nb + ((u64)p << sub);
    for (u32 j = threadIdx.x; j < nsub; j += blockDim.x) { lcur[j] = goff[j] + rel[j]; lfirst[j] = goff[j]; }
    const u32 pbase = goff[0];
    const u32 beg = pbase + pc[(gidx * slices + k0) * P + p];
    const u32 end = k1 < slices ? pbase + pc[(gidx * slices + k1) * P + p] : goff[nsub];
    __syncthreads();
    __shared__ u32 cnt[512], sbase[512], scur[512], wsum[4];
    __shared__ u32 stage[2048];
    __shared__ unsigned short stageq[2048];
    const u32 tid = threadIdx.x, lane = tid & 63, wave = tid >> 6;
    for (u32 r0 = beg; r0 < end; r0 += 2048) {
        const u32 rend = min(r0 + 2048u, end);
        unsigned long long pr[8];
        if (tid < nsub) cnt[tid] = 0;
        if (tid + 256 < nsub) cnt[tid + 256] = 0;
        __syncthreads();
#pragma unroll
        for (int j = 0; j < 8; j++) {
            u32 i = r0 + tid + j * 256;
            pr[j] = i < rend ? pairs[i] : ~0ull;
            const bool v = pr[j] != ~0ull;
            const u32 sb = (u32)(pr[j] >> 32);
            const unsigned long long act = __ballot(v);
            if (act && __ballot(v && sb != (u32)__builtin_amdgcn_readfirstlane((int)sb)) == 0 && ((act & 1ull) != 0)) {
                if (lane == 0) atomicAdd(&cnt[sb], (u32)__popcll(act));
            } else if (v) atomicAdd(&cnt[sb], 1u);
        }
        __syncthreads();
        if (nsub <= 256) {
            u32 v = tid < nsub ? cnt[tid] : 0, x = v;
#pragma unroll
            for (int d = 1; d < 64; d <<= 1) { u32 y = __shfl_up(x, d); if ((int)lane >= d) x += y; }
            if (lane == 63) wsum[wave] = x;
            __syncthreads();
            u32 before = 0;
            for (u32 w = 0; w < wave; w++) before += wsum[w];
            if (tid < nsub) { sbase[tid] = before + x - v; scur[tid] = before + x - v; }
        } else {
            const u32 v0 = cnt[2 * tid], v1 = cnt[2 * tid + 1];
            u32 x = v0 + v1;
#pragma unroll
            for (int d = 1; d < 64; d <<= 1) { u32 y = __shfl_up(x, d); if ((int)lane >= d) x += y; }
            if (lane == 63) wsum[wave] = x;
            __syncthreads();
            u32 before = 0;
            for (u32 w = 0; w < wave; w++) before += wsum[w];
            const u32 e0 = before + x - v0 - v1;
            sbase[2 * tid] = e0; scur[2 * tid] = e0;
            sbase[2 * tid + 1] = e0 + v0; scur[2 * tid + 1] = e0 + v0;
        }
        __syncthreads();
#pragma unroll
        for (int j = 0; j < 8; j++) {
            const bool v = pr[j] != ~0ull;
            const u32 sb = (u32)(pr[j] >> 32);
            const unsigned long long act = __ballot(v);
            u32 pos = 0;
            if (act && __ballot(v && sb != (u32)__builtin_amdgcn_readfirstlane((int)sb)) == 0 && ((act & 1ull) != 0)) {
                if (lane == 0) pos = atomicAdd(&scur[sb], (u32)__popcll(act));
                pos = (u32)__shfl((int)pos, 0) + (u32)__popcll(act & ((1ull << lane) - 1));
            } else if (v) pos = atomicAdd(&scur[sb], 1u);
            if (v) {
                stage[pos] = (u32)pr[j];
                stageq[pos] = (unsigned short)sb;
            }
        }
        __syncthreads();
        const u32 total = rend - r0;
        for (u32 e = tid; e < total; e += 256) {
            const u32 sb = stageq[e];
            const u32 at = lcur[sb] + (e - sbase[sb]);
            idx_out[at] = stage[e] | (at == lfirst[sb] ? MSM_IDX_FIRST : 0u);
        }
        __syncthreads();
        if (tid < nsub) lcur[tid] += cnt[tid];
        if (tid + 256 < nsub) lcur[tid + 256] += cnt[tid + 256];
    }
}

FP_DEV u32 find_segment(const u32* off, u32 total, u32 t) {
    u32 lo = 0, hi = total;
    while (hi - lo > 1) {
        u32 mid = (lo + hi) >> 1;
        if (off[mid] <= t) lo = mid; else hi = mid;
    }
    return lo;
}

template <class F>
FP_DEV aff29 load_point(const affine_t* table, u32 e, bool& is_id) {
    affine_t pk = aff_load(&table[e & MSM_IDX_MASK]);
    is_id = aff_is_identity(pk);
    aff29 q = a29_from_packed(pk);
    if (e >> 31) q.y = f29_sub(f29_zero(), q.y, F::KN);
    return q;
}

template <class CV>
__global__ __launch_bounds__(MSM_ACC_THREADS_MAX) MSM_ACC_WAVES_ATTR void k_msm_accum0(MsmGeom g, u32 total_buckets, const u32* idx, const u32* off, const u32* nrank,
                                                               const affine_t* table, xyzz29_rec* partial, const u32* geo) {
    typedef typename f29_of<typename CV::Base>::type F;
    const u32 lane = blockIdx.x * blockDim.x + threadIdx.x;
    const u32 M = off[total_buckets];
    const u32 L0 = geo[0];
    const u64 beg64 = (u64)lane * L0;
    if (beg64 >= M) return;
    const u32 beg = (u32)beg64;
    const u32 end = (u32)min((u64)M, beg64 + L0);
    u32 rec = lane + nrank[find_segment(off, total_buckets, beg)];
    u32 e = idx[beg];
    affine_t pk = aff_load(&table[e & MSM_IDX_MASK]);
    bool is_id = aff_is_identity(pk);
    aff29 q = a29_from_packed(pk);
    if (e >> 31) q.y = f29_sub(f29_zero(), q.y, F::KN);
    xyzz29 acc = x29_from_affine<F>(q, is_id);
    if (!is_id) acc.y = f29_norm(acc.y);
    u32 e_next = beg + 1 < end ? idx[beg + 1] : 0;
    for (u32 p = beg + 1; p < end; p++) {
        e = e_next;
        pk = aff_load(&table[e & MSM_IDX_MASK]);
        e_next = p + 1 < end ? idx[p + 1] : 0;
        is_id = aff_is_identity(pk);
        q = a29_from_packed(pk);
        if (e >> 31) q.y = f29_sub(f29_zero(), q.y, F::KN);
        if (e & MSM_IDX_FIRST) {
            x29_store(&partial[rec], acc);
            rec++;
            acc = x29_from_affine<F>(q, is_id);
            if (!is_id) acc.y = f29_norm(acc.y);
        } else if (!is_id) acc = x29_add_mixed<F>(acc, q);
    }
    x29_store(&partial[rec], acc);
}



template <class F>
FP_DEV void msm_emit(const xyzz29& p, jacobian_t* out, affine_t* out_affine) {
    if (out) {
        jacobian_t j = x29_to_jacobian_std<F>(p);
        f_store(&out->x, j.x); f_store(&out->y, j.y); f_store(&out->z, j.z);
    }
    if (out_affine) {
        affine_t a;
        if (f29_is_zero_slow<F>(p.zz)) { a.x = f_zero(); a.y = f_zero(); }
        else {
// ... 1 lines not shown
            a.x = f29_to_std<F>(f29_mul<F>(p.x, f29_mul<F>(ti, p.zzz)));
            a.y = f29_to_std<F>(f29_mul<F>(p.y, f29_mul<F>(ti, p.zz)));
        }
        aff_store(out_affine, a);
    }
}

#include "msm_bred.cuh"

template <class CV>
__global__ __launch_bounds__(256) void k_msm_final(MsmGeom g, const xyzz29_rec* group_sums, jacobian_t* out, affine_t* out_affine) {
    typedef f29_lat<typename f29_of<typename CV::Base>::type> F;
    __shared__ xyzz29_rec sh[64];
    const u32 bat = blockIdx.x;
    const u32 w = threadIdx.x >> 2, role = threadIdx.x & 3;
    if (g.G == 1) {
        if (threadIdx.x == 0) msm_emit<F>(x29_load(&group_sums[bat]), out ? out + bat : nullptr, out_affine ? out_affine + bat : nullptr);
        return;
    }
    xyzz29 s = x29_identity();
    if (w < g.G) s = x29_load(&group_sums[(u64)bat * g.G + w]);
    const u32 nd = w < g.G ? g.c * w : 0;
    for (u32 i = 0; i < nd; i++) s = x29_double_quad<F>(s);
    if (role == 0) x29_store(&sh[w], s);
    __syncthreads();
    for (u32 d = 32; d > 0; d >>= 1) {
        if (w < d) {
            xyzz29 x = x29_add_quad<F>(x29_load(&sh[w]), x29_load(&sh[w + d]));
            if (role == 0) x29_store(&sh[w], x);
        }
        __syncthreads();
    }
    if (threadIdx.x == 0) msm_emit<F>(x29_load(&sh[0]), out ? out + bat : nullptr, out_affine ? out_affine + bat : nullptr);
}

template <class CV>
__global__ __launch_bounds__(128) void k_msm_build_table(const affine_t* std_points, affine_t* table, u32 n, u32 c, u32 rows) {
    typedef typename CV::Base F;
    typedef typename f29_of<typename CV::Base>::type F9;
    u32 i = blockIdx.x * blockDim.x + threadIdx.x;
    if (i >= n) return;
    affine_t p = aff_load(&std_points[i]);
    xyzz_t cur = xyzz_from_affine<F>(p);
    for (u32 w = 0; w < rows; w++) {
        affine_t a = p;
        if (w > 0) {
            for (u32 k = 0; k < c; k++) cur = xyzz_double<F>(cur);
            a = xyzz_to_affine<F>(cur);
        }
        affine_t o;
        if (aff_is_identity(a)) { o.x = f_zero(); o.y = f_zero(); }
        else {
            o.x = f29_to_packed_canon<F9>(f29_from_std<F9>(a.x));
            o.y = f29_to_packed_canon<F9>(f29_from_std<F9>(a.y));
        }
        aff_store(&table[(u64)w * n + i], o);
    }
}

template <class CV>
__global__ void k_jac_to_affine(const jacobian_t* in, affine_t* out, u32 count) {
    typedef typename CV::Base F;
    u32 i = blockIdx.x * blockDim.x + threadIdx.x;
    if (i >= count) return;
    fe x = f_load(&in[i].x), y = f_load(&in[i].y), z = f_load(&in[i].z);
    affine_t a;
    if (f_is_zero(z)) { a.x = f_zero(); a.y = f_zero(); }
    else {
        typedef typename f29_of<F>::type F9;
        fe zi = f29_to_std<F9>(f29_inv_safegcd<F9>(f29_from_std<F9>(z)));
        fe zi2 = f_sqr<F>(zi);
        a.x = f_mul<F>(x, zi2);
        a.y = f_mul<F>(y, f_mul<F>(zi2, zi));
    }
    aff_store(&out[i], a);
}


static_assert(sizeof(xyzz29_rec) == MSM_REC_BYTES, "msm_plan.hpp sizes the record buffers");

static DevBuf dehalo_ctx::* const msm_ws_bufs[MSM_WS_N] = {
    &dehalo_ctx::ws_count, &dehalo_ctx::ws_counters, &dehalo_ctx::ws_bhist, &dehalo_ctx::ws_pcount, &dehalo_ctx::ws_pairs, &dehalo_ctx::ws_off, &dehalo_ctx::ws_records,
    &dehalo_ctx::ws_merge_parts, &dehalo_ctx::ws_merge_lists, &dehalo_ctx::ws_idx, &dehalo_ctx::ws_partial0, &dehalo_ctx::ws_buckets, &dehalo_ctx::ws_contrib, &dehalo_ctx::ws_tree,
    &dehalo_ctx::ws_bred_cnt, &dehalo_ctx::ws_gsums, &dehalo_ctx::ws_bsum};

template <class CV>
int run_msm_t(dehalo_ctx* ctx, const dehalo_bases* bases, const fe* d_scalars, size_t len, size_t batch, jacobian_t* d_out, hipStream_t s) {
    typedef typename CV::Scalar FS;
    if (batch == 0) return 0;
    if (len == 0) {
        HIP_TRY(ctx, hipMemsetAsync(d_out, 0, batch * sizeof(jacobian_t), s));
        return 0;
    }
    MsmTuning tuning = msm_experiment_tuning();
    tuning.sort_block = ctx->msm_sort_block; tuning.acc_block = ctx->msm_acc_block; tuning.acc_points = ctx->msm_acc_points; tuning.acc_waves = ctx->msm_acc_waves;
    tuning.acc_min_layers = ctx->msm_acc_min_layers; tuning.num_cus = ctx->num_cus;
    MsmPlan p;
    if (const char* refused = msm_plan(MsmShape{len, batch, bases->n, bases->c, bases->W, bases->precomp != 0}, tuning, &p)) return dh_fail(ctx, DEHALO_ERR_INVALID, refused);
    const MsmGeom& g = p.g;

    for (u32 i = 0; i < MSM_WS_N; i++) {
        DevBuf& b = ctx->*msm_ws_bufs[i];
        const bool grows = p.ws_bytes[i] > b.cap;
        TRY(dh_ensure(ctx, b, p.ws_bytes[i]));
        if (grows && i == MSM_WS_BRED_CNT) HIP_TRY(ctx, hipMemsetAsync(b.p, 0, b.cap, s));
    }
    const u32 tb = (u32)p.total_buckets;
    u32* count = (u32*)ctx->ws_count.p;
    u32* merge_counters = (u32*)ctx->ws_counters.p;
    u32* geo = merge_counters + MSM_MERGE_COUNTERS;
    u32* off = (u32*)ctx->ws_off.p;
    u32* nrank = (u32*)ctx->ws_records.p;
    u32* rbeg = nrank + (p.total_buckets + 1);
    u32* rend = rbeg + (p.total_buckets + 1);
    u32* merge_lists = (u32*)ctx->ws_merge_lists.p;
    u32* bh = (u32*)ctx->ws_bhist.p;
    unsigned short* bh16 = reinterpret_cast<unsigned short*>(bh + p.total_buckets * (size_t)g.slices);
    u32* pc = (u32*)ctx->ws_pcount.p;
    unsigned long long* pairs = (unsigned long long*)ctx->ws_pairs.p;
    u32* bs_i = (u32*)ctx->ws_bsum.p;
    u32* bs_t = bs_i + p.cs_a;
    u32* idx = (u32*)ctx->ws_idx.p;
    xyzz29_rec* partial0 = (xyzz29_rec*)ctx->ws_partial0.p;
    xyzz29_rec* buckets = (xyzz29_rec*)ctx->ws_buckets.p;
    xyzz29_rec* gsums = (xyzz29_rec*)ctx->ws_gsums.p;

    const void* hist_fn = p.pack16 ? (const void*)k_msm_hist<FS, true> : (const void*)k_msm_hist<FS, false>;
    if (p.lds_hist > 48 * 1024) HIP_TRY(ctx, dh_func_lds(ctx, hist_fn, (int)p.lds_hist));
    const size_t lds_part = dh_co_lds_pad(0, p.lds_part);
    HIP_TRY(ctx, dh_func_lds(ctx, (const void*)k_msm_part<FS>, (int)lds_part));
    const size_t lds_bk = dh_co_lds_pad(p.lds_bucket, 0), lds_m = dh_co_lds_pad(18 * 1024, 0), lds_b = dh_co_lds_pad(41 * 1024, 0);
    TRY(dh_co_lds_attr(ctx, (const void*)k_msm_bucket, lds_bk));
    {
        ScopedTimer t(ctx, s, DEHALO_K_MSM_SORT);
        const dim3 grid(p.sort_grid[0], p.sort_grid[1], p.sort_grid[2]);
        if (p.pack16) k_msm_hist<FS, true><<<grid, p.hist_threads, p.lds_hist, s>>>(g, d_scalars, reinterpret_cast<u32*>(bh16), pc);
        else k_msm_hist<FS, false><<<grid, p.hist_threads, p.lds_hist, s>>>(g, d_scalars, bh, pc);
        k_msm_colscan<<<p.cs_a + p.cs_b, SCAN_THREADS, 0, s>>>(g.nb, g.slices, tb, bh, p.pack16 ? bh16 : nullptr, count, p.cs_a, p.P, (u32)p.total_groups * p.P, pc, bs_i, bs_t, merge_counters);
        k_scan_offsets<<<p.cs_a, SCAN_THREADS, 0, s>>>(count, tb, bs_i, bs_t, p.cs_a, geo, (u32)p.resident, (u32)p.lmax, p.lcap, p.kmin, off, nrank, rbeg, rend,
                                                       merge_lists, p.merge_cap);
        HIP_TRY(ctx, hipGetLastError());
        k_msm_part<FS><<<grid, p.part_threads, lds_part, s>>>(g, d_scalars, off, pc, pairs, p.part_lists);
        k_msm_bucket<<<dim3(p.bucket_grid[0], p.bucket_grid[1]), p.bucket_threads, lds_bk, s>>>(g.nb, g.c, g.slices, off, bh, pc, pairs, idx, p.bslices);
        HIP_TRY(ctx, hipGetLastError());
    }
    {
        ScopedTimer t(ctx, s, DEHALO_K_MSM_ACCUMULATE);
        k_msm_accum0<CV><<<p.acc_grid, p.acc_block, p.acc_lds, s>>>(g, tb, idx, off, nrank, bases->table.p, partial0, geo);
        HIP_TRY(ctx, hipGetLastError());
    }
    {
        ScopedTimer t(ctx, s, DEHALO_K_MSM_REDUCE);
        TRY(dh_co_lds_attr(ctx, (const void*)k_msm_merge2<CV>, lds_m));
        TRY(dh_co_lds_attr(ctx, (const void*)k_msm_bred<CV>, lds_b));
        TRY(msm_stamps_arm(ctx));
        k_msm_merge2<CV><<<MERGE2_GRID, 256, lds_m, s>>>(rbeg, rend, partial0, buckets, merge_counters, merge_lists, p.merge_cap, (xyzz29_rec*)ctx->ws_merge_parts.p, tb);
        const bool fin = g.G == 1;
        k_msm_bred<CV><<<dim3(p.nblk, (u32)p.total_groups), BRED_THREADS, lds_b, s>>>(g.nb, p.bred_bb, buckets, (xyzz29_rec*)ctx->ws_contrib.p, (xyzz29_rec*)ctx->ws_tree.p, (u32*)ctx->ws_bred_cnt.p, gsums,
                                                                                     fin ? d_out : nullptr, fin ? ctx->msm_affine_out : nullptr);
        TRY(msm_stamps_report(ctx, g.nb, (u32)p.total_groups, tb, s));
        if (!fin) k_msm_final<CV><<<g.batch, 256, 0, s>>>(g, gsums, d_out, ctx->msm_affine_out);
        HIP_TRY(ctx, hipGetLastError());
    }
    return 0;
}

template <class CV>
int build_table_t(dehalo_ctx* ctx, dehalo_bases* b, const affine_t* d_std_points, hipStream_t s) {
    u32 rows = b->precomp ? b->W : 1;
    k_msm_build_table<CV><<<(u32)((b->n + 127) / 128), 128, 0, s>>>(d_std_points, b->table.p, (u32)b->n, b->c, rows);
    HIP_TRY(ctx, hipGetLastError());
    return 0;
}

template <class CV>
__global__ __launch_bounds__(64) void k_point_sum(const jacobian_t* in, u32 count, jacobian_t* out) {
    typedef f29_lat<typename f29_of<typename CV::Base>::type> F;
    const u32 lane = threadIdx.x;
    xyzz29 acc = x29_identity();
    for (u32 i = lane; i < count; i += 64) {
        fe z = f_load(&in[i].z);
        if (f_is_zero(z)) continue;
        xyzz29 p;
        f29 z29 = f29_from_std<F>(z);
        p.x = f29_from_std<F>(f_load(&in[i].x));
        p.y = f29_from_std<F>(f_load(&in[i].y));
        p.zz = f29_sqr<F>(z29);
        p.zzz = f29_mul<F>(p.zz, z29);
        acc = x29_add<F>(acc, p);
    }
    acc = x29_group_reduce<F, 64>(acc);
    if (lane == 0) {
        jacobian_t j = x29_to_jacobian_std<F>(acc);
        f_store(&out->x, j.x); f_store(&out->y, j.y); f_store(&out->z, j.z);
    }
}

template <class CV>
int point_sum_t(dehalo_ctx* ctx, const jacobian_t* d_in, uint32_t count, jacobian_t* d_out, hipStream_t s) {
    k_point_sum<CV><<<1, 64, 0, s>>>(d_in, count, d_out);
    HIP_TRY(ctx, hipGetLastError());
    return 0;
}

template <class CV>
int to_affine_t(dehalo_ctx* ctx, const jacobian_t* d_in, affine_t* d_out, uint32_t count, hipStream_t s) {
    k_jac_to_affine<CV><<<(count + 63) / 64, 64, 0, s>>>(d_in, d_out, count);
    HIP_TRY(ctx, hipGetLastError());
    return 0;
}

template <class CV>
constexpr CurveOps make_curve_ops() {
    return {&run_msm_t<CV>, &build_table_t<CV>, &to_affine_t<CV>, &point_sum_t<CV>, CV::Scalar::P};
}
```

### delay-encryption-in-halo2_amd/csrc/msm_plan.hpp

```cpp
#pragma once
#include <algorithm>
#include <cstddef>
#include <cstdint>
#include <cstdlib>

#include "experiment_env.hpp"

#ifdef __HIPCC__
#define MSM_PLAN_HD __host__ __device__
#else
#define MSM_PLAN_HD
#endif

#define MSM_SORT_THREADS 1024
#define MSM_ACC_THREADS 128
#define MSM_ACC_THREADS_MAX 768
#define MSM_MERGE_COUNTERS 8

#define MERGE2_CHUNK 512

#define MSM_IDX_FIRST 0x40000000u
#define MSM_IDX_MASK 0x3fffffffu

#define SCAN_THREADS 256

#define MSM_PART_WAVE_LDS(lists) (4 * (lists) * 4 + 512 * 8 + 512 * 2)
#define MSM_BUCKET_SLICES 4
#define MSM_BUCKET_THREADS 256
#define MSM_REC_BYTES 144

#define BRED_THREADS 256
#define BRED_BLOCK_BUCKETS 256
#define BRED_BLOCK_BUCKETS_MIN 128
#define BRED_FANIN 16
#define BRED_VMAX 17
#define BRED_CNT_PER_GROUP 32
#define MERGE2_BLOCKS_LIGHT 1024
#define MERGE2_BLOCKS_Q8 512
#define MERGE2_BLOCKS_BLOCK 512
#define MERGE2_BLOCKS_PARTS 1024
#define MERGE2_BLOCKS_COPY 256
#define MERGE2_GRID_SUMS (MERGE2_BLOCKS_PARTS + MERGE2_BLOCKS_BLOCK + MERGE2_BLOCKS_Q8 + 3 * MERGE2_BLOCKS_LIGHT)
#define MERGE2_GRID (MERGE2_GRID_SUMS + MERGE2_BLOCKS_COPY)

struct MsmGeom {
    uint32_t n;
    uint32_t table_n;
    uint32_t c;
    uint32_t W;
    uint32_t nb;
    uint32_t G;
    uint32_t batch;
    uint32_t slices;
    uint32_t L0;
    uint32_t wb;
};

MSM_PLAN_HD inline uint32_t msm_sub_bits(uint32_t c) { return c - 1 < 8 ? c - 1 : (c >= 17 ? 9u : 8u); }

#define MSM_WINDOW_MIN 4u
inline uint32_t msm_window_max(bool precomp) { return precomp ? 17u : 16u; }

inline uint32_t log2_ceil(size_t n) {
    uint32_t l = 0;
    while (((size_t)1 << l) < n) l++;
    return l;
}

inline uint32_t choose_window(size_t n) {
    uint32_t l = log2_ceil(n ? n : 1);
    if (l >= 20) return 17;
    if (l >= 19) return 16;
    if (l >= 17) return 15;
    if (l >= 10) return 13;
    return std::max<uint32_t>(6, l + 1);
}

inline uint32_t choose_window_single(size_t n) {
    uint32_t l = log2_ceil(n ? n : 1);
    if (l >= 16) return 13;
    if (l >= 12) return 10;
    return choose_window(n);
}

inline uint32_t signed_windows(const uint32_t r_words[8], uint32_t c) {
    uint64_t r1[4];
    for (int i = 0; i < 4; i++) r1[i] = (uint64_t)r_words[2 * i] | ((uint64_t)r_words[2 * i + 1] << 32);
    r1[0] -= 1;
    auto bits_at = [&](uint32_t lo, uint32_t count) -> uint64_t {
        uint64_t v = 0;
        for (uint32_t b = 0; b < count; b++) {
            uint32_t pos = lo + b;
            if (pos < 256 && ((r1[pos >> 6] >> (pos & 63)) & 1)) v |= 1ull << b;
        }
        return v;
    };
    for (uint32_t W = (254 + c - 1) / c; W <= (256 + c - 1) / c; W++) {
        if (W < 2) continue;
        const uint32_t shift = c * (W - 1);
        bool above = false;
        for (uint32_t pos = shift + c; pos < 256; pos++) above |= ((r1[pos >> 6] >> (pos & 63)) & 1) != 0;
        if (above) continue;
        const uint64_t top = bits_at(shift, c), half = 1ull << (c - 1);
        if (top + 1 <= half) return W;
        if (top == half && bits_at(shift - c, c) == 0) return W;
    }
    return (256 + c - 1) / c;
}

inline bool msm_table_fits(size_t n, uint32_t W) { return n < (1ull << 30) && (uint64_t)n * W < (1ull << 30); }

struct MsmShape {
    size_t len, batch;
    size_t table_n;
    uint32_t c, W;
    bool precomp;
};

struct MsmTuning {
    int sort_block = 1024, acc_block = 128, acc_points = 48, acc_waves = 3, acc_min_layers = 4;
    int num_cus = 256;
    bool small_slices = true;
    uint32_t hist_threads = 0, part_threads = 0;
    uint32_t bucket_slices = MSM_BUCKET_SLICES;
    bool bucket_fill = true;
    uint32_t acc_lds = 0;
    uint32_t bred_block = 0;
};

inline const MsmTuning& msm_experiment_tuning() {
    static const MsmTuning tuning = [] {
        MsmTuning t;
        auto off = [](const char* e) { return e && e[0] == '0'; };
        auto threads = [](const char* e) { const int v = e ? atoi(e) : 0; return (uint32_t)std::max(0, std::min(MSM_SORT_THREADS, v & ~63)); };
        t.small_slices = !off(DH_EXPERIMENT_ENV("DEHALO_MSM_SMALL_SLICES"));
        t.hist_threads = threads(DH_EXPERIMENT_ENV("DEHALO_MSM_HIST_THREADS"));
        t.part_threads = threads(DH_EXPERIMENT_ENV("DEHALO_MSM_PART_THREADS"));
        if (const char* e = DH_EXPERIMENT_ENV("DEHALO_MSM_BUCKET_SLICES")) { const int v = atoi(e); if (v >= 1 && v <= 16) t.bucket_slices = (uint32_t)v; }
        t.bucket_fill = !off(DH_EXPERIMENT_ENV("DEHALO_MSM_BUCKET_FILL"));
        if (const char* e = DH_EXPERIMENT_ENV("DEHALO_MSM_ACC_LDS")) t.acc_lds = (uint32_t)atoi(e);
        if (const char* e = DH_EXPERIMENT_ENV("DEHALO_MSM_BRED_BLOCK")) { const int v = atoi(e); if (v == 128 || v == 256) t.bred_block = (uint32_t)v; }
        return t;
    }();
    return tuning;
}

enum MsmWs {
    MSM_WS_COUNT, MSM_WS_COUNTERS, MSM_WS_BHIST, MSM_WS_PCOUNT, MSM_WS_PAIRS, MSM_WS_OFF, MSM_WS_RECORDS, MSM_WS_MERGE_PARTS, MSM_WS_MERGE_LISTS, MSM_WS_IDX,
    MSM_WS_PARTIAL0, MSM_WS_BUCKETS, MSM_WS_CONTRIB, MSM_WS_TREE, MSM_WS_BRED_CNT, MSM_WS_GSUMS, MSM_WS_BSUM, MSM_WS_N
};

struct MsmPlan {
    MsmGeom g;
    uint64_t total_groups, total_buckets, Mmax;
    uint32_t P;
    bool pack16;
    uint32_t hist_threads, part_threads, part_lists, sort_grid[3];
    size_t lds_hist, lds_part;
    uint32_t cs_a, cs_b;
    uint32_t bslices, bucket_threads, bucket_grid[2];
    size_t lds_bucket;
    uint32_t lcap, kmin, acc_block, acc_grid, acc_lds;
    uint64_t resident, lmax, lanes_max, nt0_max;
    uint32_t merge_cap, bred_bb, nblk;
    size_t ws_bytes[MSM_WS_N];
};

inline const char* msm_plan(const MsmShape& sh, const MsmTuning& t, MsmPlan* plan) {
    if (sh.c < MSM_WINDOW_MIN) return "msm: window below 4 bits";
    MsmPlan& p = *plan;
    p = MsmPlan{};
    MsmGeom& g = p.g;
    const size_t len = sh.len, batch = sh.batch;
    g.n = (uint32_t)len; g.table_n = (uint32_t)sh.table_n; g.c = sh.c; g.W = sh.W; g.nb = 1u << (g.c - 1);
    g.G = sh.precomp ? 1 : g.W;
    g.batch = (uint32_t)batch;
    g.L0 = 0;
    const uint32_t sort_threads = t.sort_block == 512 ? 512u : 1024u;
    g.slices = (uint32_t)std::min<size_t>(256 * (1024 / sort_threads), std::max<size_t>(1, len / (2 * sort_threads)));
    if (t.small_slices && g.G == 1 && (size_t)g.slices * batch < 128)
        g.slices = (uint32_t)std::max<size_t>(g.slices, std::min<size_t>(std::max<size_t>(1, len / 256), (128 + batch - 1) / batch));
    if ((size_t)g.nb * 4 > 128 * 1024) {
        if (g.G != 1) return "a 17-bit window needs a precomputed table";
        g.slices = (uint32_t)std::max<uint64_t>(g.slices, ((uint64_t)len * g.W + 65534) / 65535);
    }
    p.P = g.nb >> msm_sub_bits(g.c);
    {
        const uint32_t fit = std::min<uint32_t>(std::min<uint32_t>(g.W, 128 / p.P), (128u * 1024 / 4) / g.nb);
        const uint32_t fill = (uint32_t)((uint64_t)g.W * g.slices * batch / 256);
        g.wb = g.G == 1 ? g.W : std::max<uint32_t>(1, std::min<uint32_t>(fit, fill));
    }
    p.total_groups = (uint64_t)batch * g.G;
    p.total_buckets = p.total_groups * g.nb;
    p.Mmax = (uint64_t)batch * len * g.W;
    if (p.Mmax >= (1ull << 32) || p.total_buckets >= (1ull << 31)) return "batch * len * windows too large for one launch";
    const uint64_t tg = p.total_groups, tb = p.total_buckets;

    const uint32_t per_slice = (uint32_t)((len + g.slices - 1) / g.slices);
    p.pack16 = g.nb >= 2 && (uint64_t)per_slice * (g.G == 1 ? g.W : g.wb) <= 65535;
    p.lds_hist = (size_t)g.nb * (p.pack16 ? 2 : 4) * (g.G == 1 ? 1 : g.wb);
    p.hist_threads = t.hist_threads ? t.hist_threads : sort_threads;
    p.part_threads = t.part_threads ? t.part_threads : sort_threads;
    p.part_lists = (g.G == 1 ? p.P : 128u) > 128u ? 256u : 128u;
    p.lds_part = 4 * (size_t)p.part_lists + (size_t)(p.part_threads / 64) * MSM_PART_WAVE_LDS(p.part_lists);
    p.sort_grid[0] = g.slices; p.sort_grid[1] = g.G == 1 ? 1 : (g.G + g.wb - 1) / g.wb; p.sort_grid[2] = (uint32_t)batch;
    p.cs_a = ((uint32_t)tb + SCAN_THREADS - 1) / SCAN_THREADS;
    p.cs_b = ((uint32_t)tg * p.P + SCAN_THREADS - 1) / SCAN_THREADS;
    p.bslices = t.bucket_slices;
    while (t.bucket_fill && p.bslices > 1 && (uint64_t)p.P * ((g.slices + p.bslices - 1) / p.bslices) * tg < (uint64_t)t.num_cus) p.bslices >>= 1;
    p.bucket_threads = MSM_BUCKET_THREADS;
    p.bucket_grid[0] = p.P * ((g.slices + p.bslices - 1) / p.bslices); p.bucket_grid[1] = (uint32_t)tg;
    p.lds_bucket = 22 * 1024;

    p.lcap = (uint32_t)t.acc_points;
    p.kmin = (uint32_t)t.acc_min_layers;
    p.resident = (uint64_t)t.num_cus * 4 * (p.lcap ? 1 : (uint64_t)t.acc_waves) * 64;
    p.lmax = 64 * 4 / (uint64_t)t.acc_waves;
    p.acc_block = t.acc_block == MSM_ACC_THREADS_MAX ? MSM_ACC_THREADS_MAX : MSM_ACC_THREADS;
    if (p.lcap) {
        uint64_t k = 4;
        while (p.Mmax > k * p.resident * p.lcap) k += 2;
        p.lanes_max = k * p.resident + p.acc_block;
    } else {
        const uint64_t rounds_max = std::max<uint64_t>(1, (p.Mmax + p.resident * p.lmax - 1) / (p.resident * p.lmax));
        p.lanes_max = rounds_max * p.resident + p.acc_block;
    }
    p.nt0_max = p.lanes_max + tb;
    p.acc_grid = (uint32_t)((p.lanes_max + p.acc_block - 1) / p.acc_block);
    p.acc_lds = t.acc_lds;

    p.merge_cap = (uint32_t)std::max<uint64_t>(std::min<uint64_t>(tb, p.nt0_max / 2 + 1), 4 * (p.nt0_max / MERGE2_CHUNK + 2));
    const bool bred_forced = t.bred_block && g.nb / t.bred_block <= BRED_FANIN * BRED_FANIN;
    p.bred_bb = bred_forced ? t.bred_block : (g.nb <= 8192 ? 128u : 256u);
    p.nblk = std::max<uint32_t>(1, g.nb / p.bred_bb);

    const size_t REC = MSM_REC_BYTES;
    size_t* ws = p.ws_bytes;
    ws[MSM_WS_COUNT] = tb * 4;
    ws[MSM_WS_COUNTERS] = 64;
    ws[MSM_WS_BHIST] = tb * (size_t)g.slices * 6;
    ws[MSM_WS_PCOUNT] = tg * (size_t)g.slices * p.P * 4;
    ws[MSM_WS_PAIRS] = p.Mmax * 8;
    ws[MSM_WS_OFF] = (tb + 1) * 4;
    ws[MSM_WS_RECORDS] = (tb + 1) * 4 * 3;
    ws[MSM_WS_MERGE_PARTS] = (2 * (p.nt0_max / MERGE2_CHUNK) + 4) * REC;
    ws[MSM_WS_MERGE_LISTS] = (size_t)p.merge_cap * MSM_MERGE_COUNTERS * 4;
    ws[MSM_WS_IDX] = p.Mmax * 4;
    ws[MSM_WS_PARTIAL0] = p.nt0_max * REC;
    ws[MSM_WS_BUCKETS] = tb * REC;
    ws[MSM_WS_CONTRIB] = tg * std::max<size_t>(1, g.nb / BRED_BLOCK_BUCKETS_MIN) * BRED_VMAX * REC;
    ws[MSM_WS_TREE] = tg * 16 * BRED_VMAX * REC;
    ws[MSM_WS_BRED_CNT] = (size_t)tg * BRED_CNT_PER_GROUP * 4;
    ws[MSM_WS_GSUMS] = tg * REC;
    ws[MSM_WS_BSUM] = (size_t)p.cs_a * 2 * sizeof(uint32_t);
    return nullptr;
}
```

### include/dehalo.h

```cpp
#ifndef DEHALO_H
#define DEHALO_H

#include <stddef.h>
#include <stdint.h>

#ifdef __cplusplus
extern "C" {
#endif

typedef enum {
    DEHALO_OK = 0,
    DEHALO_ERR_INVALID = -1,
    DEHALO_ERR_NO_DEVICE = -2,
    DEHALO_ERR_OOM = -3,
    DEHALO_ERR_HIP = -4,
    DEHALO_ERR_UNSUPPORTED = -5,
    DEHALO_ERR_NOT_IN_TABLE = -6,
    DEHALO_ERR_SHUFFLE = -7
} dehalo_status;

typedef enum { DEHALO_CURVE_BN254_G1 = 0, DEHALO_CURVE_PALLAS = 1, DEHALO_CURVE_VESTA = 2 } dehalo_curve;
typedef enum { DEHALO_FIELD_BN254_FR = 0, DEHALO_FIELD_BN254_FQ = 1, DEHALO_FIELD_PASTA_FP = 2, DEHALO_FIELD_PASTA_FQ = 3 } dehalo_field;

typedef struct dehalo_ctx dehalo_ctx;
// ... 256 lines not shown
int dehalo_ipa_open(dehalo_ctx* ctx, const dehalo_params* params, const uint64_t* d_poly, const uint64_t blind[4], const uint64_t x3[4], dehalo_rng* rng,
                    dehalo_transcript* transcript);

int dehalo_prover_create(dehalo_ctx* ctx, dehalo_ctx* side_ctx, const dehalo_params* params, const dehalo_pk* pk, dehalo_prover** out);
int dehalo_prover_create_multi(dehalo_ctx* ctx, dehalo_ctx* side_ctx, const dehalo_params* params, const dehalo_pk* pk, uint32_t num_circuits, dehalo_prover** out);
int dehalo_prover_release(dehalo_prover* prover);
typedef enum { DEHALO_MULTIOPEN_GWC = 0, DEHALO_MULTIOPEN_SHPLONK = 1 } dehalo_multiopen;
int dehalo_prover_set_multiopen(dehalo_prover* prover, int multiopen);
size_t dehalo_prover_proof_size(const dehalo_prover* prover);
enum { DEHALO_PROOF_ADVICE_ON_DEVICE = 1, DEHALO_PROOF_ADVICE_CANONICAL = 2  };
int dehalo_create_proof(dehalo_prover* prover, const uint64_t* advice, const uint64_t* const* instances, const size_t* instance_lens, uint32_t num_instance_columns,
                        dehalo_rng* rng, dehalo_transcript* transcript, uint32_t flags);
int dehalo_create_proof_multi(dehalo_prover* prover, const uint64_t* const* advice, const uint64_t* const* instances, const size_t* instance_lens,
                              uint32_t num_instance_columns, uint32_t num_circuits, dehalo_rng* rng, dehalo_transcript* transcript, uint32_t flags);
typedef int (*dehalo_advice_fn)(void* user, uint32_t phase, const uint64_t* challenges, uint32_t num_challenges, const uint64_t** advice);
int dehalo_create_proof_phased(dehalo_prover* prover, dehalo_advice_fn fn, void* user, const uint64_t* const* instances, const size_t* instance_lens,
                               uint32_t num_instance_columns, dehalo_rng* rng, dehalo_transcript* transcript, uint32_t flags);
typedef enum { DEHALO_CHECK_GATE = 0, DEHALO_CHECK_LOOKUP = 1, DEHALO_CHECK_COPY = 2, DEHALO_CHECK_SHUFFLE = 3 } dehalo_check_kind;
typedef struct { uint32_t kind, index, row, reserved; } dehalo_check_failure;
typedef struct {
    uint64_t gate_failures, lookup_failures, copy_failures;
    uint64_t rows, lookup_inputs, cells_in_cycles;
    uint64_t written;
    uint64_t shuffle_failures, shuffle_inputs;
} dehalo_check_report;
int dehalo_check_witness(dehalo_ctx* ctx, const dehalo_pk* pk, const uint64_t* advice, const uint64_t* const* instances, const size_t* instance_lens, uint32_t num_instance_columns,
                         const uint64_t* permutation_mapping, uint32_t flags, dehalo_check_failure* failures, size_t cap, dehalo_check_report* report);
int dehalo_check_witness_challenges(dehalo_ctx* ctx, const dehalo_pk* pk, const uint64_t* advice, const uint64_t* const* instances, const size_t* instance_lens,
                                    uint32_t num_instance_columns, const uint64_t* permutation_mapping, uint32_t flags, const uint64_t* challenges, uint32_t num_challenges,
                                    dehalo_check_failure* failures, size_t cap, dehalo_check_report* report);

typedef int (*dehalo_gather_fn)(void* user, uint64_t* points, uint32_t count, const uint32_t* first, const uint32_t* num, uint32_t world);
int dehalo_prover_set_shard(dehalo_prover* prover, uint32_t rank, uint32_t world, dehalo_gather_fn gather, void* user);
int dehalo_prover_last_timings(const dehalo_prover* prover, double out[8]);
int dehalo_create_proofs(dehalo_prover* const* provers, uint32_t num_provers, const uint64_t* const* advice, uint32_t count, dehalo_rng* rngs, uint32_t flags,
                         uint8_t* const* proofs_out, size_t proof_cap, size_t* proof_lens);

typedef enum { DEHALO_CIRCUIT_DELAY_ENC = 0, DEHALO_CIRCUIT_MOD_POW = 1, DEHALO_CIRCUIT_POSE_ENC = 2 } dehalo_circuit_kind;
typedef struct {
    uint32_t circuit, k;
    uint32_t bits_len, exp_bits;
    const uint64_t *n, *x;
    uint64_t e;
    const uint64_t* message; uint32_t message_len;
    const uint64_t* key;
    uint32_t t, rate, r_f, r_p;
} dehalo_circuit_inputs;
typedef struct {
    uint64_t rsa_rows, total_rows;
    uint64_t rsa_result[128];
    uint64_t cipher[12]; uint32_t cipher_len;
} dehalo_synthesis_info;
int dehalo_synthesize(const dehalo_circuit_inputs* in, uint64_t* advice, uint64_t* fixed, uint64_t* mapping, uint8_t* const* selectors, dehalo_synthesis_info* info);
int dehalo_create_proof_circuit(dehalo_prover* prover, const dehalo_circuit_inputs* in, dehalo_synthesis_info* info, const uint64_t* const* instances,
                                const size_t* instance_lens, uint32_t num_instance_columns, dehalo_rng* rng, dehalo_transcript* transcript);
int dehalo_create_proofs_circuit(dehalo_prover* const* provers, uint32_t num_provers, const dehalo_circuit_inputs* inputs, uint32_t count, dehalo_rng* rngs,
                                 uint8_t* const* proofs_out, size_t proof_cap, size_t* proof_lens);

typedef struct {
    const uint64_t* const* columns; const uint64_t* const* sigma; uint32_t num_columns, chunk_len;
    const uint64_t* omega_powers;
    const uint64_t *beta, *gamma, *delta;
    const uint64_t* set_factors;
    const uint64_t* const* compressed_input; const uint64_t* const* compressed_table;
    const uint64_t* const* permuted_input; const uint64_t* const* permuted_table;
    uint32_t num_lookups;
} dehalo_product_inputs;
int dehalo_product_terms_device(dehalo_ctx* ctx, int field, const dehalo_product_inputs* in, size_t n, uint64_t* d_num, uint64_t* d_den, size_t stride_elems, void* stream);

typedef enum {
    DEHALO_K_MSM_ACCUMULATE = 0,
    DEHALO_K_MSM_SORT = 1,
    DEHALO_K_MSM_REDUCE = 2,
    DEHALO_K_NTT_PASS = 3,
    DEHALO_K_POLY = 4,
    DEHALO_K_EVAL_H = 5,
    DEHALO_K_COUNT = 6
} dehalo_kernel_id;
int dehalo_timing_enable(dehalo_ctx* ctx, int on);
int dehalo_timing_reset(dehalo_ctx* ctx);
int dehalo_timing_get(dehalo_ctx* ctx, int kernel_id, double* total_ms, uint64_t* count);

int dehalo_msm_last_shape(dehalo_ctx* ctx, uint32_t out[6]);

int dehalo_field_info(int field, uint64_t out[24]);

const char* dehalo_version(void);

#ifdef __cplusplus
}
#endif
#endif
```

Before: 790.3 Mpoints/s.

## Precompute packed signed digits in histogram pass and shrink sort pairs to one word

The histogram kernel now converts each scalar out of Montgomery form once, recodes it into packed signed c-bit digits and writes them to a new digit workspace, which the partition kernel reads instead of recomputing digits. Sort pairs shrink from 64-bit to 32-bit words by packing sub-bucket, sign, window and slice-local index, which forces enough slices that each holds at most 2^16 points. Wave value grouping compares a one-word XOR key before a full verification, and LDS clears and copies use 128-bit accesses. This trades an extra digit buffer write and read for less repeated scalar decoding and half the pair traffic. It also adds a bucket-slices tuning key and a last-plan query API.

```diff
diff --git a/bindings/rust/dehalo-sys/src/lib.rs b/bindings/rust/dehalo-sys/src/lib.rs
--- a/bindings/rust/dehalo-sys/src/lib.rs
+++ b/bindings/rust/dehalo-sys/src/lib.rs
@@ -482,8 +482,9 @@
     pub fn dehalo_timing_reset(ctx: *mut dehalo_ctx) -> c_int;
     pub fn dehalo_timing_get(ctx: *mut dehalo_ctx, kernel_id: c_int, total_ms: *mut f64, count: *mut u64) -> c_int;
     pub fn dehalo_msm_last_shape(ctx: *mut dehalo_ctx, out: *mut u32) -> c_int;
+    pub fn dehalo_msm_last_plan(ctx: *mut dehalo_ctx, out: *mut u32) -> c_int;
     pub fn dehalo_field_info(field: c_int, out: *mut u64) -> c_int;
     pub fn dehalo_version() -> *const c_char;
 }
 
-pub const DEHALO_SYS_FUNCTIONS: usize = 132;
+pub const DEHALO_SYS_FUNCTIONS: usize = 133;
diff --git a/delay-encryption-in-halo2_amd/_lib.py b/delay-encryption-in-halo2_amd/_lib.py
--- a/delay-encryption-in-halo2_amd/_lib.py
+++ b/delay-encryption-in-halo2_amd/_lib.py
@@ -13,7 +13,7 @@
 SYMBOLS = [
     "dehalo_version", "dehalo_ctx_create", "dehalo_ctx_create_with_priority", "dehalo_ctx_destroy", "dehalo_last_error", "dehalo_ctx_synchronize", "dehalo_download", "dehalo_upload", "dehalo_ctx_stream", "dehalo_ctx_set_tuning",
     "dehalo_bases_register", "dehalo_bases_release", "dehalo_bases_len", "dehalo_bases_info",
-    "dehalo_msm", "dehalo_msm_batch", "dehalo_msm_device", "dehalo_msm_device_affine", "dehalo_msm_last_shape", "dehalo_lookup_h_batch_device", "dehalo_product_terms_device", "dehalo_best_multiexp", "dehalo_to_affine", "dehalo_to_affine_device", "dehalo_point_sum_device",
+    "dehalo_msm", "dehalo_msm_batch", "dehalo_msm_device", "dehalo_msm_device_affine", "dehalo_msm_last_shape", "dehalo_msm_last_plan", "dehalo_lookup_h_batch_device", "dehalo_product_terms_device", "dehalo_best_multiexp", "dehalo_to_affine", "dehalo_to_affine_device", "dehalo_point_sum_device",
     "dehalo_ntt", "dehalo_ntt_device", "dehalo_intt_scaled", "dehalo_coset_ntt", "dehalo_coset_intt",
     "dehalo_intt_scaled_device", "dehalo_lagrange_to_coeff_device", "dehalo_coset_ntt_device", "dehalo_coset_intt_device",
     "dehalo_field_op", "dehalo_field_op_device", "dehalo_timing_enable", "dehalo_timing_reset", "dehalo_timing_get",
@@ -172,6 +172,8 @@
     lib.dehalo_msm_device.argtypes = [P, P, u64p, sz, sz, u64p, P]
     lib.dehalo_msm_device_affine.argtypes = [P, P, u64p, sz, sz, u64p, u64p, P]
     lib.dehalo_msm_last_shape.argtypes = [P, C.POINTER(C.c_uint32)]
+    if hasattr(lib, "dehalo_msm_last_plan"):
+        lib.dehalo_msm_last_plan.argtypes = [P, C.POINTER(C.c_uint32)]
     lib.dehalo_best_multiexp.argtypes = [P, C.c_int, u64p, u64p, sz, u64p]
     lib.dehalo_to_affine.argtypes = [P, C.c_int, u64p, sz, u64p]
     lib.dehalo_to_affine_device.argtypes = [P, C.c_int, u64p, sz, u64p, P]
@@ -450,6 +452,11 @@
         self._check(self.lib.dehalo_msm_last_shape(self.handle, out))
         return {"merge_light": out[0], "merge_32": out[1], "merge_wave": out[2], "merge_block": out[3], "points_per_lane": out[4], "pairs": out[5]}
 
+    def msm_last_plan(self) -> dict:
+        out = (C.c_uint32 * 8)()
+        self._check(self.lib.dehalo_msm_last_plan(self.handle, out))
+        return {"window_bits": out[0], "windows": out[1], "groups": out[2], "slices": out[3], "bucket_slices": out[4], "digit_words": out[5], "sort_threads": out[6], "packed": bool(out[7])}
+
     def best_multiexp(self, curve: int, scalars, affine_xy) -> np.ndarray:
         s, a = _u64(scalars, 4), _u64(affine_xy, 8)
         if s.shape[0] != a.shape[0]:
diff --git a/delay-encryption-in-halo2_amd/csrc/capi.hip b/delay-encryption-in-halo2_amd/csrc/capi.hip
--- a/delay-encryption-in-halo2_amd/csrc/capi.hip
+++ b/delay-encryption-in-halo2_amd/csrc/capi.hip
@@ -379,6 +379,11 @@
             ctx->msm_sort_block = value;
             return 0;
         }
+        if (!strcmp(key, "msm_bucket_slices")) {
+            if (value != 0 && value != 1 && value != 2 && value != 4 && value != 8 && value != MSM_BUCKET_SLICES_MAX) return dh_fail(ctx, DEHALO_ERR_INVALID, "msm_bucket_slices must be 0, 1, 2, 4, 8 or 16");
+            ctx->msm_bucket_slices = value;
+            return 0;
+        }
         if (!strcmp(key, "msm_acc_block")) {
             if (value != 128 && value != 768) return dh_fail(ctx, DEHALO_ERR_INVALID, "msm_acc_block must be 128 or 768");
             ctx->msm_acc_block = value;
@@ -1269,6 +1274,15 @@
     });
 }
 
+int dehalo_msm_last_plan(dehalo_ctx* ctx, uint32_t out[8]) {
+    if (!ctx || !out) return DEHALO_ERR_INVALID;
+    return dh_guard(ctx, [&]() -> int {
+        std::lock_guard<std::recursive_mutex> lk(ctx->mu);
+        memcpy(out, ctx->msm_last_plan, sizeof ctx->msm_last_plan);
+        return 0;
+    });
+}
+
 int dehalo_msm_last_shape(dehalo_ctx* ctx, uint32_t out[6]) {
     if (!ctx || !out) return DEHALO_ERR_INVALID;
     return dh_guard(ctx, [&]() -> int {
diff --git a/delay-encryption-in-halo2_amd/csrc/internal.hpp b/delay-encryption-in-halo2_amd/csrc/internal.hpp
--- a/delay-encryption-in-halo2_amd/csrc/internal.hpp
+++ b/delay-encryption-in-halo2_amd/csrc/internal.hpp
@@ -51,13 +51,15 @@
     std::mutex err_mu;
     std::recursive_mutex mu;
     DevBuf ws_scalars, ws_out, ws_count, ws_counters, ws_off, ws_records, ws_merge_lists, ws_merge_parts, ws_bhist, ws_pcount, ws_pairs, ws_bsum, ws_idx, ws_partial0, ws_buckets,
-        ws_contrib, ws_tree, ws_bred_cnt, ws_gsums, ws_ntt_scratch, ws_ntt_io, ws_ntt_io2, ws_fop[3], ws_tmp_bases, ws_poly[5], ws_poly_io[3], ws_evh[4], ws_lookup, ws_gfft, ws_check[3];
+        ws_contrib, ws_tree, ws_bred_cnt, ws_gsums, ws_digits, ws_ntt_scratch, ws_ntt_io, ws_ntt_io2, ws_fop[3], ws_tmp_bases, ws_poly[5], ws_poly_io[3], ws_evh[4], ws_lookup, ws_gfft, ws_check[3];
     std::vector<TwiddleEntry> twiddles;
     affine_t* msm_affine_out = nullptr;
     int msm_acc_points = 48;
     int msm_acc_waves = 3;
     int host_wait_spin_us = 400;
     int msm_acc_min_layers = 4;
+    int msm_bucket_slices = 0;
+    uint32_t msm_last_plan[8] = {};
     int msm_sort_block = 1024;
     int msm_acc_block = 128;
     int ntt_full_table_log = 0;
diff --git a/delay-encryption-in-halo2_amd/csrc/msm.cuh b/delay-encryption-in-halo2_amd/csrc/msm.cuh
--- a/delay-encryption-in-halo2_amd/csrc/msm.cuh
+++ b/delay-encryption-in-halo2_amd/csrc/msm.cuh
@@ -77,30 +77,38 @@
     }
 };
 
-FP_DEV bool wave_value_groups(const fe& s, bool active, u32 lane, u32 max_groups, u32& leader, u32& cnt, u32& rank) {
+template <int N>
+FP_DEV bool wave_value_groups(const u32 (&v)[N], bool active, u32 lane, u32 max_groups, u32& leader, u32& cnt, u32& rank) {
     unsigned long long rem = __ballot(active);
     leader = lane; cnt = 1; rank = 0;
+    u32 key = v[0];
+#pragma unroll
+    for (int w = 1; w < N; w++) key ^= v[w];
     for (u32 n = 0; rem; n++) {
         if (n == max_groups) return false;
         const int ld = __ffsll((long long)rem) - 1;
-        bool eq = active;
-#pragma unroll
-        for (int w = 0; w < 8; w++) eq &= s.v[w] == (u32)__shfl((int)s.v[w], ld);
+        const bool eq = active && key == (u32)__shfl((int)key, ld) && ((rem >> lane) & 1ull);
         const unsigned long long m = __ballot(eq);
         if (eq) { leader = (u32)ld; cnt = (u32)__popcll(m); rank = (u32)__popcll(m & ((1ull << lane) - 1)); }
         rem &= ~m;
     }
-    return true;
-}
-
-template <class FS, bool PACK16>
-__global__ __launch_bounds__(MSM_SORT_THREADS) MSM_HIST_ATTR void k_msm_hist(MsmGeom g, const fe* scalars, u32* bh, u32* pc) {
+    bool same = true;
+#pragma unroll
+    for (int w = 0; w < N; w++) same &= v[w] == (u32)__shfl((int)v[w], (int)leader);
+    return __ballot(active && !same) == 0;
+}
+
+template <class FS, bool PACK16, u32 C>
+__global__ __launch_bounds__(MSM_SORT_THREADS) MSM_HIST_ATTR void k_msm_hist(MsmGeom g, const fe* scalars, u32* bh, u32* pc, u32* dig, u64 dig_stride) {
     msm_tail_prio();
-    extern __shared__ u32 lhist[];
+    extern __shared__ __align__(16) u32 lhist[];
     const u32 bat = blockIdx.z;
     const u32 w_lo = g.G == 1 ? 0 : blockIdx.y * g.wb, w_hi = g.G == 1 ? g.W : min(g.W, w_lo + g.wb);
     const u32 ng = g.G == 1 ? 1 : w_hi - w_lo, grp0 = g.G == 1 ? 0 : w_lo;
-    for (u32 b = threadIdx.x; b < (PACK16 ? ng * g.nb / 2 : ng * g.nb); b += blockDim.x) lhist[b] = 0;
+    {
+        uint4* l4 = reinterpret_cast<uint4*>(lhist);
+        for (u32 b = threadIdx.x; b < (PACK16 ? ng * g.nb / 8 : ng * g.nb / 4); b += blockDim.x) l4[b] = make_uint4(0, 0, 0, 0);
+    }
     __syncthreads();
     const fe* sc = scalars + (u64)bat * g.n;
     const u32 per = (g.n + g.slices - 1) / g.slices;
@@ -114,16 +122,42 @@
 #pragma unroll
         for (int j = 0; j < 4; j++) {
             const bool valid = i0 + j * blockDim.x < end;
+            u32 rec[MsmDigitShape<C>::WORDS];
+            if (C) {
+                const bool nz = valid && !fe_is_zero_words(s4[j]);
+                if (__ballot(nz)) {
+                    const fe s = nz ? f_from_mont<FS>(s4[j]) : s4[j];
+                    msm_digits_pack<C>(s.v, C, nz ? g.W : 0u, rec);
+                } else {
+#pragma unroll
+                    for (u32 q = 0; q < MsmDigitShape<C>::WORDS; q++) rec[q] = 0;
+                }
+                if (valid && blockIdx.y == 0) {
+                    u32* out = dig + ((u64)bat * g.n + i0 + j * blockDim.x);
+                    const u32 words = msm_digit_words(C, g.W);
+#pragma unroll
+                    for (u32 q = 0; q < MsmDigitShape<C>::WORDS; q++)
+                        if (q < words) out[q * dig_stride] = rec[q];
+                }
+            }
             u32 gl, weight, grank;
-            const bool grouped = wave_value_groups(s4[j], valid, threadIdx.x & 63, 4, gl, weight, grank);
+            const bool grouped = wave_value_groups(s4[j].v, valid, threadIdx.x & 63, 4, gl, weight, grank);
             if (!grouped) weight = 1;
             const bool counts = grouped ? valid && (threadIdx.x & 63) == gl : valid;
-            if (counts)
-                for_each_digit<FS>(s4[j], g.c, w_lo, w_hi, [&](u32 w, u32 bucket, bool) {
-                    const u32 slot = (one ? 0u : (w - w_lo) * g.nb) + bucket;
-                    if (PACK16) atomicAdd(&lhist[slot >> 1], weight << ((slot & 1u) << 4));
-                    else atomicAdd(&lhist[slot], weight);
-                });
+            auto count_digit = [&](u32 w, u32 bucket, bool) {
+                const u32 slot = (one ? 0u : (w - w_lo) * g.nb) + bucket;
+                if (PACK16) atomicAdd(&lhist[slot >> 1], weight << ((slot & 1u) << 4));
+                else atomicAdd(&lhist[slot], weight);
+            };
+            if (C) {
+                const u32 w_end = msm_digits_end(rec);
+#pragma unroll
+                for (u32 w = 0; w < MsmDigitShape<C>::WMAX; w++) {
+                    bool neg;
+                    const u32 mag = msm_digits_get<C>(rec, C, w, &neg);
+                    if (counts && w >= w_lo && w < w_hi && w < w_end && mag != 0) count_digit(w, mag - 1, neg);
+                }
+            } else if (counts) for_each_digit<FS>(s4[j], g.c, w_lo, w_hi, count_digit);
         }
     }
     __syncthreads();
@@ -132,11 +166,13 @@
         const u64 gidx = (u64)bat * g.G + grp0 + gi;
         const u32* lh = lhist + (PACK16 ? gi * g.nb / 2 : gi * g.nb);
         if (PACK16) {
-            u32* out = bh + ((gidx * g.slices + blockIdx.x) * g.nb) / 2;
-            for (u32 w = threadIdx.x; w < g.nb / 2; w += blockDim.x) out[w] = lh[w];
+            uint4* out = reinterpret_cast<uint4*>(bh + ((gidx * g.slices + blockIdx.x) * g.nb) / 2);
+            const uint4* l4 = reinterpret_cast<const uint4*>(lh);
+            for (u32 w = threadIdx.x; w < g.nb / 8; w += blockDim.x) out[w] = l4[w];
         } else {
-            u32* out = bh + (gidx * g.slices + blockIdx.x) * g.nb;
-            for (u32 b = threadIdx.x; b < g.nb; b += blockDim.x) out[b] = lh[b];
+            uint4* out = reinterpret_cast<uint4*>(bh + (gidx * g.slices + blockIdx.x) * g.nb);
+            const uint4* l4 = reinterpret_cast<const uint4*>(lh);
+            for (u32 b = threadIdx.x; b < g.nb / 4; b += blockDim.x) out[b] = l4[b];
         }
         u32* pout = pc + (gidx * g.slices + blockIdx.x) * P;
         const u32 nsub = 1u << sub, lane = threadIdx.x & 63;
@@ -155,41 +191,43 @@
 }
 
 template <bool SRC16>
-FP_DEV u32 colscan_one(u32 nb, u32 slices, u32 total_buckets, u32* bh, const unsigned short* src16, u32* count, u32 gb) {
+FP_DEV u32 colscan_one(u32 nb, u32 slices, u32 total_buckets, u32* bh, const unsigned short* src16, u32* count, u32 gb, u32 stride) {
     if (gb >= total_buckets) return 0;
     u32 grp = gb / nb, b = gb - grp * nb;
     u32* col = bh + (u64)grp * slices * nb + b;
     const unsigned short* col16 = SRC16 ? src16 + (u64)grp * slices * nb + b : nullptr;
     u32 run = 0;
-    u32 k = 0;
+    u32 k = 0, phase = 0;
     for (; k + 16 <= slices; k += 16) {
         u32 v[16];
 #pragma unroll
         for (int j = 0; j < 16; j++) v[j] = SRC16 ? (u32)col16[(u64)(k + j) * nb] : col[(u64)(k + j) * nb];
 #pragma unroll
         for (int j = 0; j < 16; j++) {
-            col[(u64)(k + j) * nb] = run;
+            if (phase == 0) col[(u64)(k + j) * nb] = run;
+            phase = phase + 1 == stride ? 0 : phase + 1;
             run += v[j];
         }
     }
     for (; k < slices; k++) {
         u32 v = SRC16 ? (u32)col16[(u64)k * nb] : col[(u64)k * nb];
-        col[(u64)k * nb] = run;
+        if (phase == 0) col[(u64)k * nb] = run;
+        phase = phase + 1 == stride ? 0 : phase + 1;
         run += v;
     }
     if (count) count[gb] = run;
     return run;
 }
 static __global__ __launch_bounds__(SCAN_THREADS) void k_msm_colscan(u32 nb, u32 slices, u32 total_buckets, u32* bh, const unsigned short* bh16, u32* count, u32 blocks_a, u32 P,
-                                                                     u32 total_parts, u32* pc, u32* bsum_items, u32* bsum_tasks, u32* merge_counters) {
+                                                                     u32 total_parts, u32* pc, u32* bsum_items, u32* bsum_tasks, u32* merge_counters, u32 bslices) {
     msm_tail_prio();
     if (blockIdx.x == 0 && threadIdx.x < MSM_MERGE_COUNTERS) merge_counters[threadIdx.x] = 0;
     if (blockIdx.x >= blocks_a) {
-        colscan_one<false>(P, slices, total_parts, pc, nullptr, nullptr, (blockIdx.x - blocks_a) * blockDim.x + threadIdx.x);
+        colscan_one<false>(P, slices, total_parts, pc, nullptr, nullptr, (blockIdx.x - blocks_a) * blockDim.x + threadIdx.x, 1);
         return;
     }
     const u32 gb0 = blockIdx.x * blockDim.x + threadIdx.x;
-    const u32 v = bh16 ? colscan_one<true>(nb, slices, total_buckets, bh, bh16, count, gb0) : colscan_one<false>(nb, slices, total_buckets, bh, nullptr, count, gb0);
+    const u32 v = bh16 ? colscan_one<true>(nb, slices, total_buckets, bh, bh16, count, gb0, bslices) : colscan_one<false>(nb, slices, total_buckets, bh, nullptr, count, gb0, bslices);
     u32 si = v, st = v ? 1u : 0u;
 #pragma unroll
     for (int d = 32; d > 0; d >>= 1) { si += __shfl_down(si, d); st += __shfl_down(st, d); }
@@ -287,8 +325,13 @@
     }
 }
 
-template <class FS>
-__global__ __launch_bounds__(MSM_SORT_THREADS) void k_msm_part(MsmGeom g, const fe* scalars, const u32* off, const u32* pc, unsigned long long* pairs, u32 lists) {
+#define MSM_PAIR_SIGN_SHIFT (MSM_PAIR_LOCAL_BITS + MSM_PAIR_WINDOW_BITS)
+#define MSM_PAIR_SUB_SHIFT (MSM_PAIR_SIGN_SHIFT + 1)
+static_assert(MSM_PAIR_SUB_SHIFT + MSM_PAIR_SUB_BITS == 32, "a pair is one word");
+FP_DEV u32 msm_pair(u32 sub_bucket, bool neg, u32 w, u32 local) { return (sub_bucket << MSM_PAIR_SUB_SHIFT) | (neg ? 1u << MSM_PAIR_SIGN_SHIFT : 0u) | (w << MSM_PAIR_LOCAL_BITS) | local; }
+
+template <class FS, u32 C>
+__global__ __launch_bounds__(MSM_SORT_THREADS) void k_msm_part(MsmGeom g, const fe* scalars, const u32* dig, u64 dig_stride, const u32* off, const u32* pc, u32* pairs, u32 lists) {
     msm_tail_prio();
     extern __shared__ __align__(8) unsigned char part_smem[];
     const u32 bat = blockIdx.z;
@@ -297,10 +340,10 @@
     const u32 ng = g.G == 1 ? 1 : w_hi - w_lo, grp0 = g.G == 1 ? 0 : w_lo;
     const u32 PT = ng * P;
     const bool one = g.G == 1;
-    const u32 wave = threadIdx.x >> 6, lane = threadIdx.x & 63, nwaves = blockDim.x >> 6;
+    const u32 wave = threadIdx.x >> 6, lane = threadIdx.x & 63;
     u32* pcur = reinterpret_cast<u32*>(part_smem);
     unsigned char* wbase = part_smem + 4 * lists + (size_t)wave * MSM_PART_WAVE_LDS(lists);
-    unsigned long long* stage = reinterpret_cast<unsigned long long*>(wbase);
+    u32* stage = reinterpret_cast<u32*>(wbase);
     u32* lcnt = reinterpret_cast<u32*>(wbase + 512 * 8);
     u32* lbase = lcnt + lists;
     u32* lcur = lbase + lists;
@@ -312,10 +355,108 @@
         pcur[qq] = off[gidx * g.nb + (q << sub)] + pc[(gidx * g.slices + blockIdx.x) * P + q];
     }
     __syncthreads();
-    const fe* sc = scalars + (u64)bat * g.n;
     const u32 per = (g.n + g.slices - 1) / g.slices;
     const u32 beg = blockIdx.x * per, end = min(beg + per, g.n);
-    (void)nwaves;
+    auto put_grouped = [&](u32 w, u32 i, u32 bk, bool ng1, u32 gl, u32 gcnt, u32 grank) {
+        const bool put = w >= w_lo && bk != 0xffffffffu;
+        const u32 q = put ? (one ? 0u : (w - w_lo) * P) + (bk >> sub) : 0u;
+        u32 g0 = 0;
+        if (put && lane == gl) g0 = atomicAdd(&pcur[q], gcnt);
+        g0 = (u32)__shfl((int)g0, (int)gl);
+        if (put) pairs[g0 + grank] = msm_pair(bk & submask, ng1, w, i - beg);
+    };
+    auto put_staged = [&](u32 w0, u32 i, const u32 (&bk)[8], const bool (&ng8)[8]) {
+        for (u32 q = lane; q < PT; q += 64) lcnt[q] = 0;
+        __builtin_amdgcn_wave_barrier();
+#pragma unroll
+        for (int j = 0; j < 8; j++)
+            if (bk[j] != 0xffffffffu) atomicAdd(&lcnt[(one ? 0u : (w0 + j - w_lo) * P) + (bk[j] >> sub)], 1u);
+        __builtin_amdgcn_wave_barrier();
+        u32 run = 0;
+        for (u32 q0 = 0; q0 < PT; q0 += 64) {
+            const u32 q = q0 + lane;
+            const u32 v = q < PT ? lcnt[q] : 0;
+            u32 x = v;
+#pragma unroll
+            for (int d = 1; d < 64; d <<= 1) { u32 y = __shfl_up(x, d); if ((int)lane >= d) x += y; }
+            if (q < PT) {
+                lbase[q] = run + x - v; lcur[q] = run + x - v;
+                gbase[q] = v ? atomicAdd(&pcur[q], v) : 0u;
+            }
+            run += __shfl(x, 63);
+        }
+        __builtin_amdgcn_wave_barrier();
+#pragma unroll
+        for (int j = 0; j < 8; j++)
+            if (bk[j] != 0xffffffffu) {
+                const u32 q = (one ? 0u : (w0 + j - w_lo) * P) + (bk[j] >> sub);
+                const u32 pos = atomicAdd(&lcur[q], 1u);
+                stage[pos] = msm_pair(bk[j] & submask, ng8[j], w0 + j, i - beg);
+                stageq[pos] = (unsigned short)q;
+            }
+        __builtin_amdgcn_wave_barrier();
+        for (u32 e = lane; e < run; e += 64) {
+            const u32 q = stageq[e];
+            pairs[gbase[q] + (e - lbase[q])] = stage[e];
+        }
+        __builtin_amdgcn_wave_barrier();
+    };
+    if (C) {
+        constexpr u32 RW = MsmDigitShape<C>::WORDS, WMAX = MsmDigitShape<C>::WMAX;
+        const u32 words = msm_digit_words(C, g.W);
+        const u32* dcol = dig + (u64)bat * g.n;
+        u32 r_next[RW];
+        {
+            const u32 i = beg + wave * 64 + lane;
+#pragma unroll
+            for (u32 q = 0; q < RW; q++) r_next[q] = q < words && i < end ? dcol[q * dig_stride + i] : 0u;
+        }
+        for (u32 i0 = beg + wave * 64; i0 < end; i0 += blockDim.x) {
+            const u32 i = i0 + lane;
+            u32 r[RW];
+#pragma unroll
+            for (u32 q = 0; q < RW; q++) r[q] = r_next[q];
+#pragma unroll
+            for (u32 q = 0; q < RW; q++) r_next[q] = q < words && i + blockDim.x < end ? dcol[q * dig_stride + i + blockDim.x] : 0u;
+            const u32 w_end = msm_digits_end(r);
+            const bool nonzero = w_end != 0;
+            const unsigned long long actm = __ballot(nonzero);
+            if (actm == 0) continue;
+            u32 gl, gcnt, grank;
+            if (__popcll(actm) > 1 && wave_value_groups(r, nonzero, lane, 4, gl, gcnt, grank)) {
+                bool live = true;
+#pragma unroll
+                for (u32 w = 0; w < WMAX; w++) {
+                    live = live && w < w_hi && __ballot(w < w_end) != 0;
+                    if (live) {
+                        bool ng1;
+                        const u32 mag = msm_digits_get<C>(r, C, w, &ng1);
+                        put_grouped(w, i, mag - 1, ng1, gl, gcnt, grank);
+                    }
+                }
+                continue;
+            }
+            bool live = true;
+#pragma unroll
+            for (u32 w0 = 0; w0 < WMAX; w0 += 8) {
+                live = live && w0 < w_hi && __ballot(w0 < w_end) != 0;
+                if (!live || w0 + 8 <= w_lo) continue;
+                u32 bk[8];
+                bool ng8[8];
+#pragma unroll
+                for (u32 j = 0; j < 8; j++) {
+                    bk[j] = 0xffffffffu; ng8[j] = false;
+                    if (w0 + j < WMAX) {
+                        const u32 mag = msm_digits_get<C>(r, C, w0 + j, &ng8[j]);
+                        if (w0 + j >= w_lo && w0 + j < w_hi) bk[j] = mag - 1;
+                    }
+                }
+                put_staged(w0, i, bk, ng8);
+            }
+        }
+        return;
+    }
+    const fe* sc = scalars + (u64)bat * g.n;
     fe s_next;
     if (beg + wave * 64 + lane < end) s_next = f_load(&sc[beg + wave * 64 + lane]);
     for (u32 i0 = beg + wave * 64; i0 < end; i0 += blockDim.x) {
@@ -330,18 +471,12 @@
         if (nonzero) ds.template init<FS>(s_cur, g.c);
         {
             u32 gl, gcnt, grank;
-            if (__popcll(actm) > 1 && wave_value_groups(s_cur, nonzero, lane, 4, gl, gcnt, grank)) {
+            if (__popcll(actm) > 1 && wave_value_groups(s_cur.v, nonzero, lane, 4, gl, gcnt, grank)) {
                 for (u32 w = 0; w < w_hi; w++) {
                     if (__ballot(nonzero && !ds.exhausted()) == 0) break;
                     u32 bk = 0xffffffffu; bool ng1 = false;
                     if (nonzero) ds.next(bk, ng1);
-                    const bool put = nonzero && w >= w_lo && bk != 0xffffffffu;
-                    const u32 q = put ? (one ? 0u : (w - w_lo) * P) + (bk >> sub) : 0u;
-                    u32 g0 = 0;
-                    if (put && lane == gl) g0 = atomicAdd(&pcur[q], gcnt);
-                    g0 = (u32)__shfl((int)g0, (int)gl);
-                    const u32 tidx = one ? w * g.table_n + i : i;
-                    if (put) pairs[g0 + grank] = ((unsigned long long)(bk & submask) << 32) | (tidx | (ng1 ? 0x80000000u : 0u));
+                    put_grouped(w, i, bk, ng1, gl, gcnt, grank);
                 }
                 continue;
             }
@@ -359,49 +494,16 @@
                 }
             }
             if (w0 + 8 <= w_lo) continue;
-            for (u32 q = lane; q < PT; q += 64) lcnt[q] = 0;
-            __builtin_amdgcn_wave_barrier();
-#pragma unroll
-            for (int j = 0; j < 8; j++)
-                if (bk[j] != 0xffffffffu) atomicAdd(&lcnt[(one ? 0u : (w0 + j - w_lo) * P) + (bk[j] >> sub)], 1u);
-            __builtin_amdgcn_wave_barrier();
-            u32 run = 0;
-            for (u32 q0 = 0; q0 < PT; q0 += 64) {
-                const u32 q = q0 + lane;
-                const u32 v = q < PT ? lcnt[q] : 0;
-                u32 x = v;
-#pragma unroll
-                for (int d = 1; d < 64; d <<= 1) { u32 y = __shfl_up(x, d); if ((int)lane >= d) x += y; }
-                if (q < PT) {
-                    lbase[q] = run + x - v; lcur[q] = run + x - v;
-                    gbase[q] = v ? atomicAdd(&pcur[q], v) : 0u;
-                }
-                run += __shfl(x, 63);
-            }
-            __builtin_amdgcn_wave_barrier();
-#pragma unroll
-            for (int j = 0; j < 8; j++)
-                if (bk[j] != 0xffffffffu) {
-                    const u32 q = (one ? 0u : (w0 + j - w_lo) * P) + (bk[j] >> sub);
-                    const u32 pos = atomicAdd(&lcur[q], 1u);
-                    const u32 tidx = one ? (w0 + j) * g.table_n + i : i;
-                    stage[pos] = ((unsigned long long)(bk[j] & submask) << 32) | (tidx | (ng8[j] ? 0x80000000u : 0u));
-                    stageq[pos] = (unsigned short)q;
-                }
-            __builtin_amdgcn_wave_barrier();
-            for (u32 e = lane; e < run; e += 64) {
-                const u32 q = stageq[e];
-                pairs[gbase[q] + (e - lbase[q])] = stage[e];
-            }
-            __builtin_amdgcn_wave_barrier();
-        }
-    }
-}
-
-static __global__ __launch_bounds__(256) void k_msm_bucket(u32 nb, u32 c, u32 slices, const u32* off, const u32* bh, const u32* pc,
-                                                          const unsigned long long* pairs, u32* idx_out, u32 per_block) {
+            put_staged(w0, i, bk, ng8);
+        }
+    }
+}
+
+static __global__ __launch_bounds__(256) void k_msm_bucket(u32 nb, u32 c, u32 slices, const u32* off, const u32* bh, const u32* pc, const u32* pairs, u32* idx_out, u32 per_block,
+                                                          u32 per, u32 row) {
     msm_tail_prio();
-    __shared__ u32 lcur[512], lfirst[512];
+    static_assert((1u << MSM_PAIR_SUB_BITS) == 512, "a partition's sub-buckets fill lcur / lfirst / cnt");
+    __shared__ u32 lcur[512], lfirst[512], sbnd[MSM_BUCKET_SLICES_MAX];
     const u32 sub = msm_sub_bits(c), P = nb >> sub, nsub = 1u << sub;
     const u32 chunks = (slices + per_block - 1) / per_block;
     const u64 gidx = blockIdx.y;
@@ -421,6 +523,8 @@
     const u32 pbase = goff[0];
     const u32 beg = pbase + pc[(gidx * slices + k0) * P + p];
     const u32 end = k1 < slices ? pbase + pc[(gidx * slices + k1) * P + p] : goff[nsub];
+    const u32 nbnd = k1 - k0 - 1;
+    if (threadIdx.x < nbnd) sbnd[threadIdx.x] = pbase + pc[(gidx * slices + k0 + 1 + threadIdx.x) * P + p];
     __syncthreads();
     __shared__ u32 cnt[512], sbase[512], scur[512], wsum[4];
     __shared__ u32 stage[2048];
@@ -428,16 +532,16 @@
     const u32 tid = threadIdx.x, lane = tid & 63, wave = tid >> 6;
     for (u32 r0 = beg; r0 < end; r0 += 2048) {
         const u32 rend = min(r0 + 2048u, end);
-        unsigned long long pr[8];
+        u32 pr[8];
         if (tid < nsub) cnt[tid] = 0;
         if (tid + 256 < nsub) cnt[tid + 256] = 0;
         __syncthreads();
 #pragma unroll
         for (int j = 0; j < 8; j++) {
             u32 i = r0 + tid + j * 256;
-            pr[j] = i < rend ? pairs[i] : ~0ull;
-            const bool v = pr[j] != ~0ull;
-            const u32 sb = (u32)(pr[j] >> 32);
+            const bool v = i < rend;
+            pr[j] = v ? pairs[i] : 0u;
+            const u32 sb = pr[j] >> MSM_PAIR_SUB_SHIFT;
             const unsigned long long act = __ballot(v);
             if (act && __ballot(v && sb != (u32)__builtin_amdgcn_readfirstlane((int)sb)) == 0 && ((act & 1ull) != 0)) {
                 if (lane == 0) atomicAdd(&cnt[sb], (u32)__popcll(act));
@@ -469,8 +573,9 @@
         __syncthreads();
 #pragma unroll
         for (int j = 0; j < 8; j++) {
-            const bool v = pr[j] != ~0ull;
-            const u32 sb = (u32)(pr[j] >> 32);
+            const u32 ipos = r0 + tid + j * 256;
+            const bool v = ipos < rend;
+            const u32 sb = pr[j] >> MSM_PAIR_SUB_SHIFT;
             const unsigned long long act = __ballot(v);
             u32 pos = 0;
             if (act && __ballot(v && sb != (u32)__builtin_amdgcn_readfirstlane((int)sb)) == 0 && ((act & 1ull) != 0)) {
@@ -478,7 +583,10 @@
                 pos = (u32)__shfl((int)pos, 0) + (u32)__popcll(act & ((1ull << lane) - 1));
             } else if (v) pos = atomicAdd(&scur[sb], 1u);
             if (v) {
-                stage[pos] = (u32)pr[j];
+                u32 k = k0;
+                for (u32 t = 0; t < nbnd; t++) k += sbnd[t] <= ipos ? 1u : 0u;
+                const u32 tidx = ((pr[j] >> MSM_PAIR_LOCAL_BITS) & ((1u << MSM_PAIR_WINDOW_BITS) - 1)) * row + k * per + (pr[j] & ((1u << MSM_PAIR_LOCAL_BITS) - 1));
+                stage[pos] = tidx | ((pr[j] >> MSM_PAIR_SIGN_SHIFT) << 31);
                 stageq[pos] = (unsigned short)sb;
             }
         }
@@ -646,7 +754,29 @@
 static DevBuf dehalo_ctx::* const msm_ws_bufs[MSM_WS_N] = {
     &dehalo_ctx::ws_count, &dehalo_ctx::ws_counters, &dehalo_ctx::ws_bhist, &dehalo_ctx::ws_pcount, &dehalo_ctx::ws_pairs, &dehalo_ctx::ws_off, &dehalo_ctx::ws_records,
     &dehalo_ctx::ws_merge_parts, &dehalo_ctx::ws_merge_lists, &dehalo_ctx::ws_idx, &dehalo_ctx::ws_partial0, &dehalo_ctx::ws_buckets, &dehalo_ctx::ws_contrib, &dehalo_ctx::ws_tree,
-    &dehalo_ctx::ws_bred_cnt, &dehalo_ctx::ws_gsums, &dehalo_ctx::ws_bsum};
+    &dehalo_ctx::ws_bred_cnt, &dehalo_ctx::ws_gsums, &dehalo_ctx::ws_bsum, &dehalo_ctx::ws_digits};
+
+template <class FS, u32 C>
+struct MsmSortKernels {
+    static const void* hist(bool pack16) { return pack16 ? (const void*)k_msm_hist<FS, true, C> : (const void*)k_msm_hist<FS, false, C>; }
+    static const void* part() { return (const void*)k_msm_part<FS, C>; }
+    static void launch_hist(bool pack16, dim3 grid, u32 threads, size_t lds, hipStream_t s, const MsmGeom& g, const fe* scalars, u32* bh, u32* pc, u32* dig, u64 dig_stride) {
+        if (pack16) k_msm_hist<FS, true, C><<<grid, threads, lds, s>>>(g, scalars, bh, pc, dig, dig_stride);
+        else k_msm_hist<FS, false, C><<<grid, threads, lds, s>>>(g, scalars, bh, pc, dig, dig_stride);
+    }
+    static void launch_part(dim3 grid, u32 threads, size_t lds, hipStream_t s, const MsmGeom& g, const fe* scalars, const u32* dig, u64 dig_stride, const u32* off, const u32* pc, u32* pairs,
+                            u32 lists) {
+        k_msm_part<FS, C><<<grid, threads, lds, s>>>(g, scalars, dig, dig_stride, off, pc, pairs, lists);
+    }
+};
+#define MSM_SORT_DISPATCH(FS, c, use)                                        \
+    switch (msm_digits_static(c) ? (c) : 0u) {                               \
+        case 13: { typedef MsmSortKernels<FS, 13> K; use; } break;           \
+        case 15: { typedef MsmSortKernels<FS, 15> K; use; } break;           \
+        case 16: { typedef MsmSortKernels<FS, 16> K; use; } break;           \
+        case 17: { typedef MsmSortKernels<FS, 17> K; use; } break;           \
+        default: { typedef MsmSortKernels<FS, 0> K; use; } break;            \
+    }
 
 template <class CV>
 int run_msm_t(dehalo_ctx* ctx, const dehalo_bases* bases, const fe* d_scalars, size_t len, size_t batch, jacobian_t* d_out, hipStream_t s) {
@@ -659,9 +789,14 @@
     MsmTuning tuning = msm_experiment_tuning();
     tuning.sort_block = ctx->msm_sort_block; tuning.acc_block = ctx->msm_acc_block; tuning.acc_points = ctx->msm_acc_points; tuning.acc_waves = ctx->msm_acc_waves;
     tuning.acc_min_layers = ctx->msm_acc_min_layers; tuning.num_cus = ctx->num_cus;
+    if (ctx->msm_bucket_slices) { tuning.bucket_slices = (uint32_t)ctx->msm_bucket_slices; tuning.bucket_fill = false; }
     MsmPlan p;
     if (const char* refused = msm_plan(MsmShape{len, batch, bases->n, bases->c, bases->W, bases->precomp != 0}, tuning, &p)) return dh_fail(ctx, DEHALO_ERR_INVALID, refused);
     const MsmGeom& g = p.g;
+    {
+        const uint32_t lp[8] = {g.c, g.W, g.G, g.slices, p.bslices, p.digit_words, p.hist_threads, p.pack16 ? 1u : 0u};
+        memcpy(ctx->msm_last_plan, lp, sizeof lp);
+    }
 
     for (u32 i = 0; i < MSM_WS_N; i++) {
         DevBuf& b = ctx->*msm_ws_bufs[i];
@@ -681,7 +816,7 @@
     u32* bh = (u32*)ctx->ws_bhist.p;
     unsigned short* bh16 = reinterpret_cast<unsigned short*>(bh + p.total_buckets * (size_t)g.slices);
     u32* pc = (u32*)ctx->ws_pcount.p;
-    unsigned long long* pairs = (unsigned long long*)ctx->ws_pairs.p;
+    u32* pairs = (u32*)ctx->ws_pairs.p;
     u32* bs_i = (u32*)ctx->ws_bsum.p;
     u32* bs_t = bs_i + p.cs_a;
     u32* idx = (u32*)ctx->ws_idx.p;
@@ -689,23 +824,27 @@
     xyzz29_rec* buckets = (xyzz29_rec*)ctx->ws_buckets.p;
     xyzz29_rec* gsums = (xyzz29_rec*)ctx->ws_gsums.p;
 
-    const void* hist_fn = p.pack16 ? (const void*)k_msm_hist<FS, true> : (const void*)k_msm_hist<FS, false>;
+    const void *hist_fn = nullptr, *part_fn = nullptr;
+    MSM_SORT_DISPATCH(FS, g.c, (hist_fn = K::hist(p.pack16), part_fn = K::part()));
     if (p.lds_hist > 48 * 1024) HIP_TRY(ctx, dh_func_lds(ctx, hist_fn, (int)p.lds_hist));
     const size_t lds_part = dh_co_lds_pad(0, p.lds_part);
-    HIP_TRY(ctx, dh_func_lds(ctx, (const void*)k_msm_part<FS>, (int)lds_part));
+    HIP_TRY(ctx, dh_func_lds(ctx, part_fn, (int)lds_part));
+    u32* dig = (u32*)ctx->ws_digits.p;
+    u32* hist_out = p.pack16 ? reinterpret_cast<u32*>(bh16) : bh;
     const size_t lds_bk = dh_co_lds_pad(p.lds_bucket, 0), lds_m = dh_co_lds_pad(18 * 1024, 0), lds_b = dh_co_lds_pad(41 * 1024, 0);
     TRY(dh_co_lds_attr(ctx, (const void*)k_msm_bucket, lds_bk));
     {
         ScopedTimer t(ctx, s, DEHALO_K_MSM_SORT);
         const dim3 grid(p.sort_grid[0], p.sort_grid[1], p.sort_grid[2]);
-        if (p.pack16) k_msm_hist<FS, true><<<grid, p.hist_threads, p.lds_hist, s>>>(g, d_scalars, reinterpret_cast<u32*>(bh16), pc);
-        else k_msm_hist<FS, false><<<grid, p.hist_threads, p.lds_hist, s>>>(g, d_scalars, bh, pc);
-        k_msm_colscan<<<p.cs_a + p.cs_b, SCAN_THREADS, 0, s>>>(g.nb, g.slices, tb, bh, p.pack16 ? bh16 : nullptr, count, p.cs_a, p.P, (u32)p.total_groups * p.P, pc, bs_i, bs_t, merge_counters);
+        MSM_SORT_DISPATCH(FS, g.c, K::launch_hist(p.pack16, grid, p.hist_threads, p.lds_hist, s, g, d_scalars, hist_out, pc, dig, p.digit_stride));
+        k_msm_colscan<<<p.cs_a + p.cs_b, SCAN_THREADS, 0, s>>>(g.nb, g.slices, tb, bh, p.pack16 ? bh16 : nullptr, count, p.cs_a, p.P, (u32)p.total_groups * p.P, pc, bs_i, bs_t, merge_counters,
+                                                               p.bslices);
         k_scan_offsets<<<p.cs_a, SCAN_THREADS, 0, s>>>(count, tb, bs_i, bs_t, p.cs_a, geo, (u32)p.resident, (u32)p.lmax, p.lcap, p.kmin, off, nrank, rbeg, rend,
                                                        merge_lists, p.merge_cap);
         HIP_TRY(ctx, hipGetLastError());
-        k_msm_part<FS><<<grid, p.part_threads, lds_part, s>>>(g, d_scalars, off, pc, pairs, p.part_lists);
-        k_msm_bucket<<<dim3(p.bucket_grid[0], p.bucket_grid[1]), p.bucket_threads, lds_bk, s>>>(g.nb, g.c, g.slices, off, bh, pc, pairs, idx, p.bslices);
+        MSM_SORT_DISPATCH(FS, g.c, K::launch_part(grid, p.part_threads, lds_part, s, g, d_scalars, dig, p.digit_stride, off, pc, pairs, p.part_lists));
+        k_msm_bucket<<<dim3(p.bucket_grid[0], p.bucket_grid[1]), p.bucket_threads, lds_bk, s>>>(g.nb, g.c, g.slices, off, bh, pc, pairs, idx, p.bslices,
+                                                                                                (g.n + g.slices - 1) / g.slices, g.G == 1 ? g.table_n : 0u);
         HIP_TRY(ctx, hipGetLastError());
     }
     {
diff --git a/delay-encryption-in-halo2_amd/csrc/msm_digits.hpp b/delay-encryption-in-halo2_amd/csrc/msm_digits.hpp
--- /dev/null
+++ b/delay-encryption-in-halo2_amd/csrc/msm_digits.hpp
@@ -0,0 +1,91 @@
+#pragma once
+#include <cstdint>
+
+#ifndef MSM_PLAN_HD
+#ifdef __HIPCC__
+#define MSM_PLAN_HD __host__ __device__
+#else
+#define MSM_PLAN_HD
+#endif
+#endif
+#ifdef __HIPCC__
+#define MSM_DIGITS_HD __host__ __device__ __forceinline__
+#define MSM_DIGITS_UNROLL _Pragma("unroll")
+#else
+#define MSM_DIGITS_HD inline
+#define MSM_DIGITS_UNROLL
+#endif
+
+#define MSM_DIGIT_HDR_BITS 8u
+#define MSM_DIGIT_WORDS_MAX 11u
+
+MSM_PLAN_HD inline uint32_t msm_digit_words(uint32_t c, uint32_t W) { return (MSM_DIGIT_HDR_BITS + W * (c + 1) + 31) / 32; }
+MSM_PLAN_HD inline uint64_t msm_digit_stride(uint64_t scalars) { return ((scalars + 63) & ~(uint64_t)63) + 17 * 64; }
+MSM_PLAN_HD inline bool msm_digits_static(uint32_t c) { return c == 13 || c == 15 || c == 16 || c == 17; }
+
+template <uint32_t C>
+struct MsmDigitShape {
+    static constexpr uint32_t WMAX = C ? (256 + C - 1) / C : 64;
+    static constexpr uint32_t WORDS = C ? (MSM_DIGIT_HDR_BITS + WMAX * (C + 1) + 31) / 32 : MSM_DIGIT_WORDS_MAX;
+};
+
+MSM_DIGITS_HD uint32_t msm_bits_at(const uint32_t* s, uint32_t pos, uint32_t c) {
+    const uint32_t i = pos >> 5, sh = pos & 31;
+    if (i >= 8) return 0;
+    const uint32_t lo = s[i], hi = i + 1 < 8 ? s[i + 1] : 0u;
+    return (uint32_t)((((uint64_t)hi << 32) | lo) >> sh) & ((1u << c) - 1);
+}
+
+MSM_DIGITS_HD uint32_t msm_bit_length(const uint32_t* s) {
+    uint32_t bits = 0;
+    MSM_DIGITS_UNROLL
+    for (uint32_t i = 0; i < 8; i++)
+        if (s[i]) bits = 32u * i + (32u - (uint32_t)__builtin_clz(s[i]));
+    return bits;
+}
+
+MSM_DIGITS_HD void msm_rec_put(uint32_t* rec, uint32_t pos, uint32_t bits, uint32_t field) {
+    const uint32_t i = pos >> 5, sh = pos & 31;
+    rec[i] |= field << sh;
+    if (sh + bits > 32) rec[i + 1] |= field >> (32 - sh);
+}
+MSM_DIGITS_HD uint32_t msm_rec_get(const uint32_t* rec, uint32_t pos, uint32_t bits) {
+    const uint32_t i = pos >> 5, sh = pos & 31;
+    uint32_t v = rec[i] >> sh;
+    if (sh + bits > 32) v |= rec[i + 1] << (32 - sh);
+    return v & ((1u << bits) - 1);
+}
+
+template <uint32_t C>
+MSM_DIGITS_HD void msm_digits_pack(const uint32_t* s, uint32_t c_rt, uint32_t W, uint32_t* rec) {
+    const uint32_t c = C ? C : c_rt;
+    const uint32_t words = C ? MsmDigitShape<C>::WORDS : msm_digit_words(c, W);
+    MSM_DIGITS_UNROLL
+    for (uint32_t j = 0; j < MsmDigitShape<C>::WORDS; j++)
+        if (j < words) rec[j] = 0;
+    const uint32_t bits = msm_bit_length(s);
+    if (bits == 0) return;
+    const uint32_t w_end = (bits + c - 1) / c + 1;
+    rec[0] = w_end < W ? w_end : W;
+    const uint32_t half = 1u << (c - 1);
+    uint32_t carry = 0;
+    MSM_DIGITS_UNROLL
+    for (uint32_t w = 0; w < MsmDigitShape<C>::WMAX; w++)
+        if (w < W) {
+            const uint32_t raw = msm_bits_at(s, w * c, c) + carry;
+            const bool neg = raw > half;
+            carry = neg ? 1u : 0u;
+            const uint32_t mag = neg ? (1u << c) - raw : raw;
+            msm_rec_put(rec, MSM_DIGIT_HDR_BITS + w * (c + 1), c + 1, mag | (carry << c));
+        }
+}
+
+MSM_DIGITS_HD uint32_t msm_digits_end(const uint32_t* rec) { return rec[0] & ((1u << MSM_DIGIT_HDR_BITS) - 1); }
+
+template <uint32_t C>
+MSM_DIGITS_HD uint32_t msm_digits_get(const uint32_t* rec, uint32_t c_rt, uint32_t w, bool* neg) {
+    const uint32_t c = C ? C : c_rt;
+    const uint32_t f = msm_rec_get(rec, MSM_DIGIT_HDR_BITS + w * (c + 1), c + 1);
+    *neg = (f >> c) != 0;
+    return f & ((1u << c) - 1);
+}
diff --git a/delay-encryption-in-halo2_amd/csrc/msm_plan.hpp b/delay-encryption-in-halo2_amd/csrc/msm_plan.hpp
--- a/delay-encryption-in-halo2_amd/csrc/msm_plan.hpp
+++ b/delay-encryption-in-halo2_amd/csrc/msm_plan.hpp
@@ -12,6 +12,8 @@
 #define MSM_PLAN_HD
 #endif
 
+#include "msm_digits.hpp"
+
 #define MSM_SORT_THREADS 1024
 #define MSM_ACC_THREADS 128
 #define MSM_ACC_THREADS_MAX 768
@@ -26,6 +28,10 @@
 
 #define MSM_PART_WAVE_LDS(lists) (4 * (lists) * 4 + 512 * 8 + 512 * 2)
 #define MSM_BUCKET_SLICES 4
+#define MSM_BUCKET_SLICES_MAX 16
+#define MSM_PAIR_LOCAL_BITS 16
+#define MSM_PAIR_WINDOW_BITS 6
+#define MSM_PAIR_SUB_BITS 9
 #define MSM_BUCKET_THREADS 256
 #define MSM_REC_BYTES 144
 
@@ -147,7 +153,7 @@
 
 enum MsmWs {
     MSM_WS_COUNT, MSM_WS_COUNTERS, MSM_WS_BHIST, MSM_WS_PCOUNT, MSM_WS_PAIRS, MSM_WS_OFF, MSM_WS_RECORDS, MSM_WS_MERGE_PARTS, MSM_WS_MERGE_LISTS, MSM_WS_IDX,
-    MSM_WS_PARTIAL0, MSM_WS_BUCKETS, MSM_WS_CONTRIB, MSM_WS_TREE, MSM_WS_BRED_CNT, MSM_WS_GSUMS, MSM_WS_BSUM, MSM_WS_N
+    MSM_WS_PARTIAL0, MSM_WS_BUCKETS, MSM_WS_CONTRIB, MSM_WS_TREE, MSM_WS_BRED_CNT, MSM_WS_GSUMS, MSM_WS_BSUM, MSM_WS_DIGITS, MSM_WS_N
 };
 
 struct MsmPlan {
@@ -159,6 +165,8 @@
     size_t lds_hist, lds_part;
     uint32_t cs_a, cs_b;
     uint32_t bslices, bucket_threads, bucket_grid[2];
+    uint32_t digit_words;
+    uint64_t digit_stride;
     size_t lds_bucket;
     uint32_t lcap, kmin, acc_block, acc_grid, acc_lds;
     uint64_t resident, lmax, lanes_max, nt0_max;
@@ -168,6 +176,8 @@
 
 inline const char* msm_plan(const MsmShape& sh, const MsmTuning& t, MsmPlan* plan) {
     if (sh.c < MSM_WINDOW_MIN) return "msm: window below 4 bits";
+    if (sh.W > (1u << MSM_PAIR_WINDOW_BITS)) return "msm: more than 64 windows";
+    static_assert(MSM_PAIR_SUB_BITS + 1 + MSM_PAIR_WINDOW_BITS + MSM_PAIR_LOCAL_BITS == 32, "a pair is one word");
     MsmPlan& p = *plan;
     p = MsmPlan{};
     MsmGeom& g = p.g;
@@ -184,6 +194,7 @@
         if (g.G != 1) return "a 17-bit window needs a precomputed table";
         g.slices = (uint32_t)std::max<uint64_t>(g.slices, ((uint64_t)len * g.W + 65534) / 65535);
     }
+    g.slices = (uint32_t)std::max<uint64_t>(g.slices, ((uint64_t)len + (1u << MSM_PAIR_LOCAL_BITS) - 1) >> MSM_PAIR_LOCAL_BITS);
     p.P = g.nb >> msm_sub_bits(g.c);
     {
         const uint32_t fit = std::min<uint32_t>(std::min<uint32_t>(g.W, 128 / p.P), (128u * 1024 / 4) / g.nb);
@@ -206,11 +217,13 @@
     p.sort_grid[0] = g.slices; p.sort_grid[1] = g.G == 1 ? 1 : (g.G + g.wb - 1) / g.wb; p.sort_grid[2] = (uint32_t)batch;
     p.cs_a = ((uint32_t)tb + SCAN_THREADS - 1) / SCAN_THREADS;
     p.cs_b = ((uint32_t)tg * p.P + SCAN_THREADS - 1) / SCAN_THREADS;
-    p.bslices = t.bucket_slices;
+    p.bslices = std::min<uint32_t>(std::max<uint32_t>(1, t.bucket_slices), MSM_BUCKET_SLICES_MAX);
     while (t.bucket_fill && p.bslices > 1 && (uint64_t)p.P * ((g.slices + p.bslices - 1) / p.bslices) * tg < (uint64_t)t.num_cus) p.bslices >>= 1;
     p.bucket_threads = MSM_BUCKET_THREADS;
     p.bucket_grid[0] = p.P * ((g.slices + p.bslices - 1) / p.bslices); p.bucket_grid[1] = (uint32_t)tg;
     p.lds_bucket = 22 * 1024;
+    p.digit_words = msm_digits_static(g.c) ? msm_digit_words(g.c, g.W) : 0u;
+    p.digit_stride = msm_digit_stride((uint64_t)batch * len);
 
     p.lcap = (uint32_t)t.acc_points;
     p.kmin = (uint32_t)t.acc_min_layers;
@@ -253,5 +266,6 @@
     ws[MSM_WS_BRED_CNT] = (size_t)tg * BRED_CNT_PER_GROUP * 4;
     ws[MSM_WS_GSUMS] = tg * REC;
     ws[MSM_WS_BSUM] = (size_t)p.cs_a * 2 * sizeof(uint32_t);
+    ws[MSM_WS_DIGITS] = (size_t)p.digit_words * p.digit_stride * 4;
     return nullptr;
 }
diff --git a/include/dehalo.h b/include/dehalo.h
--- a/include/dehalo.h
+++ b/include/dehalo.h
@@ -362,6 +362,7 @@
 int dehalo_timing_get(dehalo_ctx* ctx, int kernel_id, double* total_ms, uint64_t* count);
 
 int dehalo_msm_last_shape(dehalo_ctx* ctx, uint32_t out[6]);
+int dehalo_msm_last_plan(dehalo_ctx* ctx, uint32_t out[8]);
 
 int dehalo_field_info(int field, uint64_t out[24]);
 
```

Result: no change. 792.1 Mpoints/s, median of 2 (+0.2%).
